# JuliaQuantumControl/GRAPE.jl

Measured on AMD Instinct MI355X. Metric: GRAPE gradient evals/sec (N=64, 1000 steps, 128 traj), higher is better.
Workload: dtype f64

## Files before the change

### grape.jl_amd/api.py

```python
from __future__ import annotations

import ctypes as C
import os
import subprocess
import sys

import numpy as np

_HERE = os.path.dirname(os.path.abspath(__file__))
_CSRC = os.path.join(_HERE, "csrc")
_LIBNAME = "libgrape_hip.so"

J_T_SM, J_T_SS, J_T_RE = 0, 1, 2
GRAD_GRADGEN, GRAD_TAYLOR = 0, 1
PROP_EXP, PROP_SERIES = 0, 1
ABI_VERSION = 7

STATUS = {0: "GRAPE_OK", -1: "GRAPE_ERR_INVALID", -2: "GRAPE_ERR_HIP", -3: "GRAPE_ERR_CHI_NORM",
          -4: "GRAPE_ERR_SINGULAR", -5: "GRAPE_ERR_TAYLOR", -6: "GRAPE_ERR_NO_CONTROLS", -7: "GRAPE_ERR_AGAIN",
          -8: "GRAPE_ERR_HOST"}

EXPORTS = ["grape_create", "grape_destroy", "grape_eval", "grape_forward", "grape_backward",
           "grape_forward_device", "grape_backward_device", "grape_check", "grape_get_propagator",
           "grape_get_tau_grads", "grape_get_storage", "grape_get_timings", "grape_reset_timings", "grape_get_work", "grape_get_cert_table",
# ... 384 lines not shown

    def hvp_forward(self, V, final_states=False):
        v, nv = self._hvp_dirs(V)
        dtau = np.empty((nv, self.K), dtype=np.complex128)
        dsums = np.empty(nv, dtype=np.complex128)
        dpsi = np.empty((nv, self.K, self.N), dtype=np.complex128) if final_states else None
        self._chk(self._lib.grape_hvp_forward(self._h, nv, v.ctypes.data, dtau.ctypes.data, dsums.ctypes.data,
                                              dpsi.ctypes.data if final_states else None))
        if v.ndim == 1:
            dtau, dsums, dpsi = dtau[0], dsums[0], (dpsi[0] if final_states else None)
        return (dtau, dsums, dpsi) if final_states else (dtau, dsums)

    def hvp_backward(self, f_total, df_total):
        one = np.ndim(df_total) == 0
        df = np.ascontiguousarray(df_total, dtype=np.complex128)
        if np.ndim(df_total) > 1 or df.size == 0:
            raise ValueError(f"df_total must be a complex scalar or [nv] with nv >= 1, got {np.shape(df_total)}")
        nv = df.size
        out = np.empty((nv, self.L * self.N_T))
        f = np.array([complex(f_total).real, complex(f_total).imag], dtype=np.float64)
        self._chk(self._lib.grape_hvp_backward(self._h, nv, f.ctypes.data, df.ctypes.data, out.ctypes.data))
        return out[0] if one else out

    def hvp_backward_chi(self, chi, dchi):
        chi = np.ascontiguousarray(chi, dtype=np.complex128)
        d = np.ascontiguousarray(dchi, dtype=np.complex128)
        if chi.shape != (self.K, self.N):
            raise ValueError(f"chi must be [K, N] = [{self.K}, {self.N}], got {chi.shape}")
        if d.ndim not in (2, 3) or d.shape[-2:] != (self.K, self.N) or d.size == 0:
            raise ValueError(f"dchi must be [K, N] = [{self.K}, {self.N}] or [nv, {self.K}, {self.N}] with nv >= 1, got {d.shape}")
        nv = 1 if d.ndim == 2 else d.shape[0]
        out = np.empty((nv, self.L * self.N_T))
        self._chk(self._lib.grape_hvp_backward_chi(self._h, nv, chi.ctypes.data, d.ctypes.data, out.ctypes.data))
        return out[0] if d.ndim == 2 else out

    def set_tlist(self, tlist):
        t = np.ascontiguousarray(tlist, dtype=np.float64)
        if t.shape != (self.N_T + 1,):
            raise ValueError(f"tlist must have N_T + 1 = {self.N_T + 1} points, got {t.shape}")
        self._chk(self._lib.grape_set_tlist(self._h, t.ctypes.data))
        self._tlist = t

    def forward_device(self, d_pulsevals_ptr, d_out_ptr, stream=0):
        self._chk(self._lib.grape_forward_device(self._h, d_pulsevals_ptr, d_out_ptr, stream))

    def backward_device(self, d_f_ptr, d_G_ptr, stream=0):
        self._chk(self._lib.grape_backward_device(self._h, d_f_ptr, d_G_ptr, stream))

    def set_fused_sweeps(self, on=True):
        return bool(self._lib.grape_set_fused_sweeps(self._h, int(bool(on))))

    def check(self, stream=0):
        self._chk(self._lib.grape_check(self._h, stream))

    def propagator(self, k, n):
        out = np.empty((self.N, self.N), dtype=np.complex128)
        self._chk(self._lib.grape_get_propagator(self._h, k, n, out.ctypes.data))
        return out.T.copy()

    def tau_grads(self):
        out = np.empty((self.K, self.L, self.N_T), dtype=np.complex128)
        self._chk(self._lib.grape_get_tau_grads(self._h, out.ctypes.data))
        return out

    def storage(self, which=0):
        out = np.empty((self.K, self.N_T + 1, self.N), dtype=np.complex128)
        self._chk(self._lib.grape_get_storage(self._h, which, out.ctypes.data))
        return out

    def timings(self):
        ms = np.full(8, -1.0)
        self._lib.grape_get_timings(self._h, ms.ctypes.data, 8)
        out = dict(zip(["expm", "forward", "backward", "deriv", "reduce", "total"], ms[:6].tolist()))
        if ms[6] >= 0.0:
            out["host_enqueue"] = float(ms[6])
        if ms[7] >= 0.0:
            out["gradient_allreduce_us"] = float(ms[7]) * 1e3
        return out

    def reset_timings(self):
        self._chk(self._lib.grape_reset_timings(self._h))

    def work(self):
        w = np.zeros(20)
        self._lib.grape_get_work(self._h, w.ctypes.data, 20)
        return dict(cells=w[0], squarings=w[1], flop_expm=w[2], flop_deriv=w[3], deriv_orders=w[4],
                    pivoted_cells=w[5], expm_cells=w[6], series_terms=w[7], series_steps=w[8],
                    t18_mfma_flop=w[9], t18_squarings=w[10], t18_cells=w[11], matrix_free_fallback=w[12], t16_cells=w[13],
                    asm_kernel=w[14], asm_deriv_kernel=w[15], asm_blocked_products=w[16],
                    walk_steps=w[17], scan_block=w[18], t16_certified=w[19])

    def cert_table(self):
        dims = np.zeros(3, np.int32)
        self._chk(self._lib.grape_get_cert_table(self._h, dims.ctypes.data, None, None))
        KC, n8, n6 = (int(x) for x in dims)
        coef, exps = np.zeros((KC, n8 + n6)), np.zeros(n8 + n6, np.int32)
        if n8 + n6:
            self._chk(self._lib.grape_get_cert_table(self._h, dims.ctypes.data, coef.ctypes.data, exps.ctypes.data))
        ex = np.stack([(exps >> (4 * l)) & 15 for l in range(self.L)], axis=1) if n8 + n6 else np.zeros((0, self.L), np.int32)
        return coef[:, :n8], coef[:, n8:], ex


def liouvillian(H, cops=()):
    H = np.asarray(H, dtype=np.complex128)
    d = H.shape[0]
    if H.shape != (d, d):
        raise ValueError(f"H must be [d, d], got {H.shape}")
    eye = np.eye(d)
    heff = H.copy()
    for A in cops:
        A = np.asarray(A, dtype=np.complex128)
        heff = heff - 0.5j * (A.conj().T @ A)
    out = np.kron(eye, heff) - np.kron(heff.conj(), eye)
    for A in cops:
        A = np.asarray(A, dtype=np.complex128)
        out = out + 1j * np.kron(A.conj(), A)
    return out


class GrapeHipOpen(GrapeHip):

    def __init__(self, H0, Hc, cops, tlist, rho0, target, weights=None, functional=J_T_SM, shape=None, K_total=None,
                 device=0, chi_min_norm=0.0, prop_tolerance=0.0):
        self._lib = load_library()
        H0 = np.asarray(H0)
        if H0.ndim != 3 or H0.shape[1] != H0.shape[2]:
            raise ValueError(f"H0 must be [K, d, d], got {H0.shape}")
        K, N = H0.shape[0], H0.shape[1]
        Hc = np.asarray(Hc)
        per_traj = Hc.ndim == 4
        if Hc.ndim not in (3, 4) or Hc.shape[-2:] != (N, N) or (per_traj and Hc.shape[0] != K):
            raise ValueError(f"Hc must be [L, d, d] or [K, L, d, d] with d = {N}, K = {K}, got {Hc.shape}")
        L = Hc.shape[1] if per_traj else Hc.shape[0]
        tlist = np.ascontiguousarray(tlist, dtype=np.float64)
        if tlist.ndim != 1 or len(tlist) < 2:
            raise ValueError("tlist must hold at least two time points")
        N_T = len(tlist) - 1
        if weights is not None and np.shape(weights) != (K,):
            raise ValueError(f"weights must be [K] = [{K}], got {np.shape(weights)}")
        cops = None if cops is None or np.size(cops) == 0 else np.asarray(cops)
        cops_per_traj = cops is not None and cops.ndim == 4
        if cops is not None and (cops.ndim not in (3, 4) or cops.shape[-2:] != (N, N) or (cops_per_traj and cops.shape[0] != K)):
            raise ValueError(f"cops must be [J, d, d] or [K, J, d, d] with d = {N}, K = {K}, got {cops.shape}")
        self.N, self.L, self.K, self.N_T = N, L, K, N_T
        self.J = 0 if cops is None else cops.shape[-3]
        self.K_total = K if K_total is None else int(K_total)
        self.functional = functional
        self.prop_method = PROP_EXP
        self.lambda_b = 0.0
        self._H0 = _c128(np.swapaxes(H0, -1, -2), (K, N, N))
        self._Hc = _c128(np.swapaxes(Hc, -1, -2))
        self._cops = None if cops is None else _c128(np.swapaxes(cops, -1, -2))
        self._psi0 = _c128(np.swapaxes(np.asarray(rho0), -1, -2), (K, N, N))
        self._target = None if target is None else _c128(np.swapaxes(np.asarray(target), -1, -2), (K, N, N))
        self._tlist = tlist
        self._weights = None if weights is None else np.ascontiguousarray(weights, dtype=np.float64)
        self._shape = None if shape is None else np.ascontiguousarray(shape, dtype=np.float64).reshape(L, N_T)
        p = _Problem()
        p.abi_version = ABI_VERSION
        p.N, p.L, p.K, p.K_total, p.N_T = N, L, K, self.K_total, N_T
        p.functional, p.gradient_method, p.hc_per_traj, p.device = functional, GRAD_GRADGEN, int(per_traj), device
        p.tlist = self._tlist.ctypes.data
        p.H0 = self._H0.ctypes.data
        p.Hc = self._Hc.ctypes.data
        p.shape = None if self._shape is None else self._shape.ctypes.data
        p.psi0 = self._psi0.ctypes.data
        p.target = None if self._target is None else self._target.ctypes.data
        p.weights = None if self._weights is None else self._weights.ctypes.data
        p.chi_min_norm = chi_min_norm
        p.prop_method, p.prop_tolerance = PROP_EXP, float(prop_tolerance)
        d = _Lindblad()
        d.J, d.cops_per_traj = self.J, int(cops_per_traj)
        d.cops = None if self._cops is None else self._cops.ctypes.data
# ... 114 lines not shown
```

### grape.jl_amd/csrc/grape_hip.hip

```cpp
#include "../../include/grape_hip.h"
#include "grape_kernels.hip.h"
#include "grape_t18_coeffs.h"
#include "grape_econ_coeffs.h"
#include "grape_large.hip.h"
#include "grape_series.hip.h"
#include "grape_cheby.hip.h"
#include "grape_timegrad.hip.h"
#include "grape_lindblad.hip.h"
#include "grape_lindblad_tg.hip.h"
#include "grape_hvp.hip.h"
#include "grape_hvp_split.hip.h"
#include "grape_lindblad_hvp.hip.h"
#include "grape_lindblad_batch.hip.h"
#include "grape_lindblad_rc.hip.h"
#include "grape_devmem.h"
#include "grape_cert.hip.h"

#include <rccl/rccl.h>
#include <dlfcn.h>
#include <mutex>

#include <algorithm>
#include <chrono>
#include <cmath>
// ... 15 lines not shown
        *err = std::string("host-side C++ exception caught at the C boundary: ") + what;
    } catch (...) {
    }
    return -8;
}
#define GRAPE_BARRIER(errptr)                                                                                   \
    catch (const std::bad_alloc &) { return barrier_fail((errptr), "std::bad_alloc (out of host memory)"); }    \
    catch (const std::exception &e) { return barrier_fail((errptr), e.what()); }                                \
    catch (...) { return barrier_fail((errptr), "unknown exception"); }

void test_throw_point(const char *where) {
    const char *hk = getenv("GRAPE_TEST_HOOKS");
    if (!(hk && atoi(hk) == 1)) return;
    const char *t = getenv("GRAPE_TEST_THROW"), *at = getenv("GRAPE_TEST_THROW_AT");
    if (!t || strcmp(at ? at : "early", where)) return;
    if (!strcmp(t, "bad_alloc")) throw std::bad_alloc();
    throw std::runtime_error(t);
}

constexpr int kRing = 64;
constexpr int kPhases = 6;
struct Phase { hipEvent_t e0, e1; bool used; };

}

struct OpenCtx;

struct grape_handle {
    grape_problem p{};
    int N = 0, NP = 0, NT = 0, L = 0, K = 0, K_total = 0, N_T = 0;
    int device = 0;
    hipStream_t stream = nullptr;
    double *d_H0f = nullptr, *d_Hcf = nullptr, *d_H0t = nullptr, *d_Hct = nullptr;
    double *d_H0p = nullptr, *d_Hcp = nullptr, *d_vecs = nullptr;
    double *d_H0q = nullptr, *d_Hcq = nullptr, *d_park2 = nullptr;
    double *d_H0q3 = nullptr, *d_Hcq3 = nullptr, *d_H0p3 = nullptr, *d_Hcp3 = nullptr;
    int deriv4_blocks = 0;
    double *d_park3 = nullptr;
    int deriv3_blocks = 0, deriv3_wpt = 0;
    bool deriv3_h0g = false;
    bool deriv3_general = false;
    int deriv2 = 0, deriv2_maxm = 0;
    bool deriv_stream = false;
    bool deriv_stream_never = false;
    int deriv_blocks = 0;
    bool large = false;
    int chunk = 0;
    double *d_lg[9] = {nullptr, nullptr, nullptr, nullptr, nullptr, nullptr, nullptr, nullptr, nullptr};
    double *d_dinv = nullptr;
    int *d_scell = nullptr;
    double *d_colpart = nullptr;
    bool lg_form2 = false;
    double *d_normpart = nullptr;
    double *d_dts = nullptr, *d_shape = nullptr, *d_weights = nullptr;
    double2 *d_psi0 = nullptr, *d_target = nullptr;
    double *d_eps = nullptr;
    double2 *d_U = nullptr, *d_fw = nullptr, *d_bw = nullptr, *d_tg = nullptr;
    double *d_ret = nullptr;
    double *d_out = nullptr;
    double *d_f = nullptr, *d_G = nullptr, *d_rho = nullptr;
    int *d_flags = nullptr;
    int *d_cellflag = nullptr;
    int KC = 0;
    bool herm = false;
    bool herm_ctrl = false;
    bool t18 = false;
    bool t18_small = true;
    bool t16 = true;
    double *d_gram = nullptr;
    int *d_celllist = nullptr;
    double *d_cert = nullptr;
    int *d_cert_exp = nullptr;
    int cert_n8 = 0, cert_n6 = 0;
    bool asm16 = false;
    bool asm16p = false;
    double *d_dte = nullptr;
    bool asm18gp = false;
    bool asm18g = false;
    int *d_wgtab = nullptr, *d_prog = nullptr, *d_splan = nullptr;
    double2 *d_xinit = nullptr;
    int asm_blocks = 0;
    int last_walk_fuse = 0;
    bool asm_sq = true;
    int asm_walk = 0;
    bool foreign_stream = false;
    bool credit_pending = false;
    std::vector<double> bal;
    std::vector<double> bal_stage_chi, bal_stage_xi;
    double *d_Sf = nullptr;
    bool expm_persist = true;
    int expm_lds_pad_kb = 0;
    bool test_hooks = false;
    bool lg_asm = true;
    bool deriv3_asm = true;
    bool taylor_check = true;
    bool no_target = false;
    std::vector<int> cls;
    int *d_cls = nullptr, *d_rep = nullptr;
    int coop_S = 0;
    int *d_xcc_sw = nullptr;
    int coop_rpw = 0, coop_nw = 0;
    double2 *d_Dt = nullptr, *d_xi = nullptr;
    double *d_wq = nullptr, *d_gb = nullptr;
    bool have_gb = false;
    const double2 *xi_user = nullptr;
    double lambda_user = 0.0;
    unsigned long long *d_stats = nullptr;
    double *h_pin = nullptr;
    DeviceBufs mem;
    size_t h_pin_doubles = 0;
    Phase ph[kRing][kPhases]{};
    long n_fwd = 0, n_bwd = 0;
    std::string err;
    bool have_forward = false, in_eval = false;
    double chi_min_norm = 1e-100, taylor_tol = 1e-16;
    int taylor_max_order = 100;
    bool fuse = false;
    bool fuse_on = true;
    bool want_bw = true;
    bool bw_done = false;
    bool bw_unit = false;
    bool z_valid = false;
    double *d_inv_tnorm = nullptr, *d_ones = nullptr;
    double2 *d_z = nullptr;
    bool scan16 = false;
    int scan_Bk = 0, scan_NB = 0;
    double2 *d_scanF = nullptr, *d_scan_fw = nullptr, *d_scan_bw = nullptr;
    int num_cus = 256;
    bool series = false;
    bool u_fallback = false;
    double *d_rb = nullptr;
    double series_tol = 1e-17, series_theta = 3.0;
    double *d_n1 = nullptr;
    double2 *d_gpark = nullptr;
    int *d_morder = nullptr;
    int maxp = 0;
    int *d_batchflag = nullptr;
    bool deriv_econ = false;
    const double *d_econ_pairs = nullptr;
    int *d_celldeg = nullptr;
    double sub_theta = 0.0;
    int sq_plan = 2;
    double2 *d_xch = nullptr;
    int *d_xcc = nullptr;
    int cheby_S = 0, cheby_round = 0, cheby_pair = 0;
    double2 *d_chi_in = nullptr;
    std::vector<grape_handle *> shards;
    std::vector<int> shard_lo;
    std::vector<int> shard_dev;
    bool use_rccl = false;
    void *comm_set = nullptr;
    std::vector<double *> d_red;
    bool rccl_fwd_checked = false, rccl_bwd_checked = false;
    hipEvent_t ar0 = nullptr, ar1 = nullptr;
    double allreduce_ms = 0.0;
    long allreduce_calls = 0;
    std::vector<double> h_multi;
    bool multi_threads = true;
    double host_enqueue_ms = 0.0;
    long host_enqueue_calls = 0;
    bool graph_ok = false, capturing = false;
    hipGraph_t graph = nullptr;
    hipGraphExec_t graph_exec = nullptr;
    bool graph_fuse_on = true;
    bool graph_bw_unit = false, graph_z_valid = false, graph_credit = false;
    long n_eval = 0;
// ... 40 lines not shown
#define HIPCHK(h, expr)                                                                         \
    do {                                                                                        \
        hipError_t _e = (expr);                                                                 \
        if (_e != hipSuccess) {                                                                 \
            (h)->err = std::string(#expr) + ": " + hipGetErrorString(_e);                       \
            return GRAPE_ERR_HIP;                                                               \
        }                                                                                       \
    } while (0)

template <typename Layout>
int group_reserve(grape_handle *h, GroupStore &g, int want, size_t per, double budget_cap, const char *call, const char *unit_word,
                  const char *env_name, int *units, Layout &&layout, bool *grown = nullptr) {
    hipError_t e = g.plan(want, per, budget_cap, units);
    if (e != hipSuccess) { h->err = std::string("hipMemGetInfo(&free_b, &total_b): ") + hipGetErrorString(e); return GRAPE_ERR_HIP; }
    const GroupStore::Grow r = g.grow(*units, h->stream, layout, &e);
    if (grown) *grown = r == GroupStore::Grow::grown;
    if (r == GroupStore::Grow::sync_failed) { h->err = std::string("hipStreamSynchronize(h->stream): ") + hipGetErrorString(e); return GRAPE_ERR_HIP; }
    if (r == GroupStore::Grow::alloc_failed) {
        h->err = GroupStore::oom_message(call, *units, unit_word, per, env_name);
        (void)hipGetLastError();
        return GRAPE_ERR_HIP;
    }
    return GRAPE_OK;
}

int copy_info(const double *info, int len, double *out, int n) {
    const int m = std::max(0, std::min(n, len));
    for (int i = 0; i < m; ++i) out[i] = info[i];
    return m;
}

struct LdsLimit {
    size_t set[64] = {0};
    hipError_t ensure(const void *fn, int dev, size_t bytes) {
        size_t &cur = set[((unsigned)dev) % 64u];
        if (bytes <= cur) return hipSuccess;
        hipError_t e = hipFuncSetAttribute(fn, hipFuncAttributeMaxDynamicSharedMemorySize, (int)bytes);
        if (e == hipSuccess) cur = bytes;
        return e;
    }
};

size_t expm_lds_bytes(int NT) {
    const int total = NT == 1 ? ExpmLds<1>::TOTAL : NT == 2 ? ExpmLds<2>::TOTAL : NT == 3 ? ExpmLds<3>::TOTAL : ExpmLds<4>::TOTAL;
    return sizeof(double) * (size_t)total;
}

template <int NT>
hipError_t launch_expm(const ExpmArgs &a, bool herm, hipStream_t s, int persistent_blocks = 0, int lds_pad_kb = 0) {
    static LdsLimit lim_fast, lim_piv, lim_herm, lim_pers, lim_persh;
    const size_t lds = expm_lds_bytes(NT) + (size_t)lds_pad_kb * 1024;
    int dev = 0;
    hipGetDevice(&dev);
    {
        hipError_t e = lim_fast.ensure((const void *)expm_pade_kernel<NT, false>, dev, lds);
        if (e == hipSuccess) e = lim_piv.ensure((const void *)expm_pade_kernel<NT, true>, dev, lds);
        if (e == hipSuccess && NT >= 3) e = lim_herm.ensure((const void *)expm_pade_kernel<NT, false, NT >= 3>, dev, lds);
        if (e != hipSuccess) return e;
    }
    hipError_t e = hipMemsetAsync(a.cellflag, 0, (size_t)a.K * a.N_T * sizeof(int), s);
    if (e != hipSuccess) return e;
    if (NT == 4 && persistent_blocks > 0) {
        hipError_t ep = lim_pers.ensure((const void *)expm_persistent_kernel<NT, false>, dev, lds);
        if (ep == hipSuccess) ep = lim_persh.ensure((const void *)expm_persistent_kernel<NT, NT == 4>, dev, lds);
        if (ep != hipSuccess) return ep;
        if (herm) hipLaunchKernelGGL((expm_persistent_kernel<NT, NT == 4>), dim3(persistent_blocks), dim3(NT * 64), lds, s, a);
        else hipLaunchKernelGGL((expm_persistent_kernel<NT, false>), dim3(persistent_blocks), dim3(NT * 64), lds, s, a);
    } else
    if (herm && NT >= 3)
        hipLaunchKernelGGL((expm_pade_kernel<NT, false, NT >= 3>), dim3(a.K * a.N_T), dim3(NT * 64), lds, s, a);
    else
        hipLaunchKernelGGL((expm_pade_kernel<NT, false>), dim3(a.K * a.N_T), dim3(NT * 64), lds, s, a);
    hipLaunchKernelGGL((expm_pade_kernel<NT, true>), dim3(std::min(a.K * a.N_T, 1024)), dim3(NT * 64), lds, s, a);
    return hipGetLastError();
}

extern "C" int grape_t18_launch(int NT, int herm, int t16, const void *args, size_t args_size, void *stream, int blocks);
extern "C" const double *grape_econ_pairs(void);
extern "C" int grape_t16p_asm_launch(const void *args, size_t args_size, int *verdict, void *stream, int blocks,
                                     const void *const *walk, int fuse, int K, const double *dte);
extern "C" int grape_t18g_asm_launch(const void *args, size_t args_size, int *verdict, void *stream, int blocks,
                                     const void *const *walk, int fuse, int K, const double *dte);
extern "C" int grape_t16_asm_launch(const void *args, size_t args_size, int *verdict, void *stream, int blocks,
                                    const void *const *walk, int fuse, int K);
extern "C" int grape_t18_batch_launch(int herm, const void *args, size_t args_size, const void *strides, size_t strides_size,
                                      int sets, void *stream, int blocks);
extern "C" void grape_t16_walks(int KC, int N_T, int nblk, int *tab);
extern "C" int grape_t16_credit_launch(const void *args, size_t args_size, void *stream);
static bool deriv3_fits(int NT, int L, bool h0_general = false) {
    const size_t tile = (size_t)2 * 16 * 17 * sizeof(double), mat = (size_t)(NT * (NT + 1) / 2) * tile;
    if (h0_general) return NT >= 3 && NT <= 4 && L >= 1 && L <= 2 && (size_t)NT * NT * tile + (size_t)L * mat <= 160 * 1024;
    return L >= 1 && L <= 8 && (size_t)(1 + L) * mat <= 160 * 1024;
}
extern "C" int grape_deriv3_launch(int NT, const void *d2args, size_t d2size, const double *H0f, const double *Hcf, int wpt,
                                   int skip_if_flagged, int h0_general, int use_asm, void *stream, int blocks);
extern "C" int grape_lg_asm_launch(const void *k, size_t size, unsigned blocks, void *stream);
extern "C" int grape_deriv4_launch(int NP, const void *d2args, size_t d2size, const double *H0q3, const double *Hcq3, const double *H0p3,
                                   const double *Hcp3, void *stream, int blocks);
#ifdef GRAPE_DIAG
extern "C" void grape_t18_set_stamps(unsigned long long *d_stamps, void *stream);
#endif

template <int CPL>
hipError_t launch_coop(const SweepArgs &a, bool backward, int S, int rpw, int nw, hipStream_t s) {
    hipError_t e;
    if (a.xcc) {
        e = hipMemsetAsync(a.xcc, 0xFF, (size_t)a.K * 32 * sizeof(int), s);
        if (e != hipSuccess) return e;
    }
    e = hipMemsetAsync((void *)a.store, 0xFF, (size_t)a.K * (a.N_T + 1) * 64 * CPL * sizeof(double2), s);
    if (e != hipSuccess) return e;
    const dim3 grid(8 * ((a.K + 7) / 8) * S), block(64 * nw);
#define COOP_CASE(NW_, RPW_)                                                                                          \
    if (nw == NW_ && rpw == RPW_) {                                                                                   \
        if (backward) hipLaunchKernelGGL((sweep_coop_kernel<CPL, RPW_, NW_, true>), grid, block, 0, s, a, S);         \
        else hipLaunchKernelGGL((sweep_coop_kernel<CPL, RPW_, NW_, false>), grid, block, 0, s, a, S);                 \
        return hipGetLastError();                                                                                     \
    }
    COOP_CASE(4, 1) COOP_CASE(8, 1) COOP_CASE(16, 1) COOP_CASE(16, 2) COOP_CASE(16, 4)
#undef COOP_CASE
    return hipErrorInvalidValue;
}

static bool g_sweep_wg32 = false;
template <int NP>
hipError_t launch_sweep(const SweepArgs &a, bool backward, hipStream_t s);
template <int NP>
hipError_t launch_sweep_pair(const SweepArgs &af, const SweepArgs &ab, hipStream_t s);

template <int NT>
hipError_t launch_scan_block(const ScanArgs &sa, hipStream_t s) {
    static LdsLimit lim;
    constexpr int NP = 16 * NT;
    const size_t lds = (size_t)2 * 2 * NP * (NP + 2) * sizeof(double);
    int dev = 0;
    hipGetDevice(&dev);
    hipError_t e = lim.ensure((const void *)scan_block_kernel<NT>, dev, lds);
    if (e != hipSuccess) return e;
    hipLaunchKernelGGL((scan_block_kernel<NT>), dim3((unsigned)(sa.KC * sa.NB)), dim3(64 * NT), lds, s, sa);
    return hipGetLastError();
}

hipError_t launch_scan(grape_handle *h, const SweepArgs *af, const SweepArgs *ab, bool blocks, hipStream_t s) {
    const int NB = h->scan_NB, Bk = h->scan_Bk, NP = h->NP;
    const SweepArgs &any = af ? *af : *ab;
    hipError_t e = hipSuccess;
    if (blocks) {
        if (NP == 16) {
            Scan16Args sa{};
            sa.U = any.U; sa.F = h->d_scanF; sa.KC = h->KC; sa.N_T = any.N_T; sa.Bk = Bk; sa.NB = NB;
            hipLaunchKernelGGL(scan16_block_kernel, dim3((unsigned)(h->KC * NB)), dim3(64), 0, s, sa);
            e = hipGetLastError();
        } else {
            ScanArgs sa{};
            sa.U = any.U; sa.F = h->d_scanF; sa.KC = h->KC; sa.N_T = any.N_T; sa.Bk = Bk; sa.NB = NB;
            e = NP == 32 ? launch_scan_block<2>(sa, s) : NP == 48 ? launch_scan_block<3>(sa, s) : launch_scan_block<4>(sa, s);
        }
        if (e != hipSuccess) return e;
    }
    SweepArgs cf{}, cb{};
    if (af) { cf = *af; cf.U = h->d_scanF; cf.N_T = NB; cf.store = h->d_scan_fw; cf.resume = nullptr; }
    if (ab) { cb = *ab; cb.U = h->d_scanF; cb.N_T = NB; cb.store = h->d_scan_bw; cb.resume = nullptr; }
    if (af && ab) e = NP == 16 ? launch_sweep_pair<16>(cf, cb, s) : NP == 32 ? launch_sweep_pair<32>(cf, cb, s)
                      : NP == 48 ? launch_sweep_pair<48>(cf, cb, s) : launch_sweep_pair<64>(cf, cb, s);
    else {
        const SweepArgs &c1 = af ? cf : cb;
        const bool bw = !af;
// ... 778 lines not shown
    return ra;
}

hipError_t launch_cheby(grape_handle *h, const SweepArgs *sf, const SweepArgs *sb, hipStream_t s) {
    const int NP = h->NP, S = h->cheby_S, K = h->K;
    const size_t lds = sizeof(double) * ((size_t)2 * 16 * (NP + 2) + 2 * (size_t)NP + CHEBY_MAXT + 2);
    static LdsLimit lim;
    {
        hipError_t e = lim.ensure((const void *)cheby_coop_kernel, h->device, lds);
        if (e != hipSuccess) return e;
    }
    hipLaunchKernelGGL(cheby_arm_kernel, dim3(256), dim3(256), 0, s, (unsigned long long *)h->d_xch, (size_t)2 * K * 4 * NP * 2);
    hipError_t e = hipGetLastError();
    if (e != hipSuccess) return e;
    e = hipMemsetAsync(h->d_xcc, 0xFF, (size_t)2 * K * 32 * sizeof(int), s);
    if (e != hipSuccess) return e;
    auto fill = [&](ChebyArgs &c, const SweepArgs &sa, bool backward) {
        c.s = sa;
        c.H0 = backward ? h->d_H0t : h->d_H0f;
        c.Hc = backward ? h->d_Hct : h->d_Hcf;
        c.eps = h->d_eps; c.shape = h->d_shape; c.dts = h->d_dts; c.rb = h->d_rb; c.stats = h->d_stats;
        c.xch = h->d_xch + (backward ? (size_t)K * 4 * NP : 0);
        c.xcc = h->d_xcc + (backward ? (size_t)K * 32 : 0);
        c.tol = h->series_tol;
        c.L = h->L; c.hc_per_traj = h->p.hc_per_traj; c.NP = NP; c.herm = h->herm ? 1 : 0;
    };
    for (int k0 = 0; k0 < K; k0 += h->cheby_round) {
        const int kn = std::min(h->cheby_round, K - k0);
        ChebyArgs cf{}, cb{};
        if (sf) { fill(cf, *sf, false); cf.k0 = k0; cf.kn = kn; }
        if (sb) { fill(cb, *sb, true); cb.k0 = k0; cb.kn = kn; }
        const int nb = 8 * ((kn + 7) / 8) * S;
        if (sf && sb) hipLaunchKernelGGL(cheby_coop_kernel, dim3(2 * nb), dim3(256), lds, s, cf, cb, S, nb);
        else if (sf) { cb = cf; cb.kn = 0; hipLaunchKernelGGL(cheby_coop_kernel, dim3(nb), dim3(256), lds, s, cf, cb, S, nb); }
        else { cf = cb; hipLaunchKernelGGL(cheby_coop_kernel, dim3(nb), dim3(256), lds, s, cf, cb, S, 0); }
        e = hipGetLastError();
        if (e != hipSuccess) return e;
    }
    return hipSuccess;
}

int status_from_flags(grape_handle *h, int flags) {
    if (flags & 32) {
        h->err = "the squaring plan of the blocked exponential was too short for this evaluation; the plan has been "
                 "adapted: repeat the call (the host-pointer entry points do so themselves)";
        return GRAPE_ERR_AGAIN;
    }
    if (flags & 1) { h->err = "Pade denominator numerically singular in at least one cell"; return GRAPE_ERR_SINGULAR; }
    if (flags & 64) { h->err = "exponential: a generator H_kn dt is not finite (NaN or overflow)"; return GRAPE_ERR_SINGULAR; }
    if (flags & 2) {
        h->err = "The chi state of at least one trajectory has norm < chi_min_norm (optimize.jl:1021-1025)";
        return GRAPE_ERR_CHI_NORM;
    }
    if (flags & 8) { h->err = "cooperative sweep: a sibling workgroup did not arrive (spin limit reached)"; return GRAPE_ERR_HIP; }
    if (flags & 16) {
        h->err = "matrix-free propagator: the series of exp(-i H dt) did not converge within the order limit";
        return GRAPE_ERR_TAYLOR;
    }
    if (flags & 4) {
        const bool cut_at_the_limit = h->NP < 48 || h->taylor_max_order <= 64;
        const bool one_term = h->p.gradient_method == GRAPE_GRAD_TAYLOR && h->taylor_max_order <= 1;
        if ((h->taylor_check || !cut_at_the_limit) && !one_term) {
            h->err = h->taylor_check ? "taylor_grad_step! did not converge within max_order iterations (optimize.jl:644-648)"
                                     : "taylor_grad_check_convergence = false with taylor_max_order > 64: a series of this evaluation was "
                                       "still unconverged at the 64 terms the series kernels of N > 32 hold";
            return GRAPE_ERR_TAYLOR;
        }
    }
    return GRAPE_OK;
}

int multi_create(grape_handle **out, const grape_problem *p);
struct HandleGuard {
    grape_handle *h;
    explicit HandleGuard(grape_handle *h_) : h(h_) {}
    HandleGuard(const HandleGuard &) = delete;
    HandleGuard &operator=(const HandleGuard &) = delete;
    ~HandleGuard() { if (h) { grape_destroy(h); (void)hipGetLastError(); } }
    grape_handle *release() { grape_handle *r = h; h = nullptr; return r; }
};
thread_local const std::vector<double> *tl_forced_bal = nullptr;
int multi_fail(grape_handle *h, grape_handle *c, int rc);
int backward_device_impl(grape_handle *h, const double *d_f, double *d_G, hipStream_t s, const double2 *d_chi);
double open_lambda_b(const grape_handle *h);

double functional_from_sums(const grape_handle *h, const double *sums) {
    const double Kt = (double)h->K_total;
    double J;
    if (h->p.functional == GRAPE_J_T_SM) J = 1.0 - (sums[0] * sums[0] + sums[1] * sums[1]) / (Kt * Kt);
    else if (h->p.functional == GRAPE_J_T_SS) J = 1.0 - sums[2] / Kt;
    else J = 1.0 - sums[3] / Kt;
    if (h->open) { if (open_lambda_b(h) != 0.0) J += open_lambda_b(h) * sums[4]; }
    else if (h->p.Dpen && h->p.lambda_b != 0.0) J += h->p.lambda_b * sums[4];
    return J;
}


}

struct OpenCtx {
    int J = 0, cops_per_traj = 0, Kj = 1, Kc = 1;
    double *d_H0 = nullptr, *d_Hc = nullptr, *d_Dc = nullptr, *d_A = nullptr, *d_AdA = nullptr, *d_rho0 = nullptr, *d_target = nullptr,
           *d_chi = nullptr, *d_weights = nullptr, *d_eps = nullptr, *d_shape = nullptr, *d_dts = nullptr, *d_rb = nullptr,
           *d_store = nullptr, *d_ws = nullptr, *d_out = nullptr, *d_f = nullptr, *d_rho = nullptr, *d_G = nullptr;
    double2 *d_tg = nullptr;
    int *d_flags = nullptr;
    unsigned long long *d_stats = nullptr;
    DeviceBufs mem;
    hipEvent_t ev[2] = {nullptr, nullptr};
    double ms_fwd = 0.0, ms_bwd = 0.0;
    long n_fwd = 0, n_bwd = 0;
    std::vector<double> out;
    std::vector<double> stage;
    bool have_bwd = false;
    enum { TG_NONE, TG_NO_GRADIENT, TG_FORWARD_ONLY, TG_READY, TG_FAILED, TG_NEW_GRID, TG_BATCH, TG_NEW_COST, TG_RUNNING_COST };
    int tg_state = TG_NONE;
    bool tg_chi_user = false;
    size_t ws_mats = 0;
    double2 *d_tq = nullptr;
    double *d_dJdt = nullptr;
    enum { HV_NONE, HV_READY, HV_FAILED, HV_NEW_GRID, HV_BATCH, HV_NEW_COST };
    int hv_state = HV_NONE;
    struct HvpStore {
        GroupStore store;
        double *d_hvV = nullptr, *d_hvws = nullptr, *d_hvds = nullptr, *d_hvout = nullptr;
        double2 *d_hvdtau = nullptr, *d_hvdcoef = nullptr, *d_hvtg = nullptr;
        unsigned long long *d_hvstats = nullptr;
        double info[7] = {0., 0., 0., 0., 0., 0., 0.};
    } hv;
    struct BatchStore {
        GroupStore store;
        double *d_obeps = nullptr, *d_obstore = nullptr, *d_obws = nullptr, *d_obout = nullptr, *d_obrho = nullptr, *d_obG = nullptr;
        double2 *d_obtg = nullptr;
        int *d_obflags = nullptr;
        unsigned long long *d_obstats = nullptr;
        double info[7] = {0., 0., 0., 0., 0., 0., 0.};
    } ob;
    bool rc_set = false;
    int rc_per_traj = 0;
    double rc_lambda = 0.0;
    double *d_Xi = nullptr, *d_wq = nullptr, *d_gb = nullptr, *d_xi_user = nullptr;
    std::vector<double> tlist;
};

namespace {

template <typename T>
hipError_t open_alloc(OpenCtx *o, T **p, size_t n) { return o->mem.alloc(p, std::max<size_t>(n, 1)); }

double open_lambda_b(const grape_handle *h) { return h->open->rc_set ? h->open->rc_lambda : 0.0; }

void open_destroy(grape_handle *h) {
    OpenCtx *o = h->open;
    hipSetDevice(h->device);
    if (h->stream) hipStreamSynchronize(h->stream);
    o->hv.store.release(); o->ob.store.release(); o->mem.release();
    for (hipEvent_t e : o->ev)
        if (e) hipEventDestroy(e);
    if (h->stream) hipStreamDestroy(h->stream);
    delete o;
    delete h;
}

void open_to_planar(const double *src, int N, int NP, double *dst) {
    std::fill(dst, dst + 2 * (size_t)NP * NP, 0.0);
    for (int j = 0; j < N; ++j)
// ... 1132 lines not shown
        std::vector<double> rb((size_t)K + (size_t)Kc * L);
        const bool rigorous = h->herm && h->series && h->large;
        auto bound_of = [&](const double *m) { return rigorous ? herm_norm2_bound(m, N) : norm2_estimate(m, N); };
        const int nops = K + Kc * L;
        auto op_ptr = [&](int q) { return q < K ? p->H0 + 2 * (size_t)q * nn : p->Hc + 2 * (size_t)(q - K) * nn; };
        if (rigorous && nops > 1) {
            parallel_for(nops, [&](int q) { rb[q] = bound_of(op_ptr(q)); });
        } else {
            for (int q = 0; q < nops; ++q) rb[q] = bound_of(op_ptr(q));
        }
        CCHK(h->mem.alloc(&h->d_rb, rb.size()));
        CCHK(hipMemcpy(h->d_rb, rb.data(), rb.size() * 8, hipMemcpyHostToDevice));
        const char *envd = getenv("GRAPE_DERIV_THETA");
        h->sub_theta = p->gradient_method == GRAPE_GRAD_GRADGEN ? (envd ? atof(envd) : 4.0) : 0.0;
        CCHK(h->mem.alloc(&h->d_batchflag, (size_t)2 * K * ((N_T + 15) / 16)));
        CCHK(hipMemset(h->d_batchflag, 0, (size_t)2 * K * ((N_T + 15) / 16) * sizeof(int)));
    }
    if (h->series) {
        const char *env = getenv("GRAPE_SERIES_THETA");
        if (env && atof(env) > 0) h->series_theta = atof(env);
        const char *envp = getenv("GRAPE_SERIES_PARK");
        const size_t bytes = (size_t)K * N_T * 32 * NP * 16;
        size_t free_p = 0, total_p = 0;
        if (const char *envb = getenv("GRAPE_U_BUDGET_GB")) free_p = (size_t)(atof(envb) * 1073741824.0);
        else if (hipMemGetInfo(&free_p, &total_p) != hipSuccess) free_p = (size_t)-1;
        if (NP >= 48 && !h->large && h->deriv2 && h->series_tol <= h->taylor_tol && bytes <= ((size_t)24 << 30) &&
            (double)bytes <= 0.5 * (double)free_p && !(envp && atoi(envp) == 0)) {
            h->maxp = 32;
            CCHK(h->mem.alloc(&h->d_gpark, (size_t)K * N_T * h->maxp * NP));
            CCHK(h->mem.alloc(&h->d_morder, (size_t)K * N_T));
            CCHK(hipMemset(h->d_morder, 0xFF, (size_t)K * N_T * sizeof(int)));
        }
    }
    CCHK(h->mem.alloc(&h->d_fw, (size_t)K * (N_T + 1) * NP));
    CCHK(h->mem.alloc(&h->d_bw, (size_t)K * (N_T + 1) * NP));
    {
        const char *envs = getenv("GRAPE_SCAN16");
        if (const char *envs2 = getenv("GRAPE_SCAN")) envs = envs2;
        { const char *env1w = getenv("GRAPE_SWEEP1W"); g_sweep_wg32 = env1w && atoi(env1w) == 0; }
        const bool forced = envs && atoi(envs) != 0;
        const int kmax = NP == 16 ? 96 : NP == 32 ? 64 : NP == 48 ? 48 : 24;
        if (NP <= 64 && !h->series && !h->large && !(envs && atoi(envs) == 0) && N_T >= 8 && (forced || (h->KC <= kmax && N_T >= 64))) {
            const double t2 = NP == 16 ? 0.22 : NP == 32 ? 1.1 : 1.8, t1 = NP == 16 ? 0.45 : NP == 32 ? 3.3 : NP == 48 ? 7.3 : 13.5;
            const double slots = NP == 16 ? 16.0 * h->num_cus : (double)h->num_cus;
            int best = 4;
            double best_t = 1e300;
            for (int Bk = 4; Bk <= 64 && Bk < std::max(N_T, 5); Bk += (Bk < 16 ? 2 : 4)) {
                const int NBq = (N_T + Bk - 1) / Bk;
                const double t = std::ceil((double)h->KC * NBq / slots) * Bk * t1 + (NBq + Bk) * t2;
                if (t < best_t) { best_t = t; best = Bk; }
            }
            if (const char *envb = getenv("GRAPE_SCAN16_BK")) best = std::max(2, atoi(envb));
            h->scan_Bk = std::min(best, N_T);
            h->scan_NB = (N_T + h->scan_Bk - 1) / h->scan_Bk;
            CCHK(h->mem.alloc(&h->d_scanF, (size_t)h->KC * h->scan_NB * NP * NP));
            CCHK(h->mem.alloc(&h->d_scan_fw, (size_t)K * (h->scan_NB + 1) * NP));
            CCHK(h->mem.alloc(&h->d_scan_bw, (size_t)K * (h->scan_NB + 1) * NP));
            h->scan16 = true;
        }
    }
    CCHK(h->mem.alloc(&h->d_tg, (size_t)K * L * N_T));
    CCHK(h->mem.alloc(&h->d_ret, (size_t)2 * K + 8 + (size_t)L * N_T + 4 + (size_t)GRAPE_STAT_SHARDS * GRAPE_STAT_SLOTS));
    h->d_out = h->d_ret;
    h->d_G = h->d_ret + (size_t)2 * K + 8;
    h->d_flags = (int *)(h->d_G + (size_t)L * N_T);
    h->d_stats = (unsigned long long *)(h->d_G + (size_t)L * N_T + 4);
    CCHK(h->mem.alloc(&h->d_f, 2)); CCHK(h->mem.alloc(&h->d_rho, (size_t)K));
    CCHK(h->mem.alloc(&h->d_cellflag, (size_t)K * N_T));
    bool sf_per_cell_ok = false;
    const char *envp16 = getenv("GRAPE_EXPM_ASM16P");
    const bool p_direct = p->hc_per_traj && (h->herm ? L <= 4 : L <= 2) && !(envp16 && atoi(envp16) == 0);
    if (p->hc_per_traj && !p_direct && h->t18 && !h->large && !h->series && h->NT == 4) {
        size_t free_b = 0, total_b = 0;
        CCHK(hipMemGetInfo(&free_b, &total_b));
        const char *envs = getenv("GRAPE_SF_PER_CELL");
        sf_per_cell_ok = !(envs && atoi(envs) == 0) && 2.0 * (double)h->KC * N_T * NP * NP * 16.0 + 8e9 < (double)free_b;
    }
    const bool sf_shape_ok = !p->hc_per_traj || p_direct || sf_per_cell_ok;
    h->asm16 = h->asm16 && h->t16 && h->t18 && h->herm && !h->large && !h->series && h->NT == 4 && sf_shape_ok && (long)K * N_T < (1L << 28);
    h->asm18g = h->asm18g && h->t18 && !h->herm && !h->large && !h->series && h->NT == 4 && sf_shape_ok && (long)K * N_T < (1L << 28);
    h->asm16p = h->asm16 && p_direct;
    h->asm18gp = h->asm18g && p_direct;
    {
        const char *enve = getenv("GRAPE_DERIV_ECON");
        const bool lg_ok = h->large && h->t18 && h->herm && !h->series;
        const bool t16c_ok = h->t16 && h->t18 && h->herm && !h->large && !h->series && (h->NT >= 3 || (h->NT == 2 && h->t18_small));
        h->deriv_econ = (h->asm16 || lg_ok || t16c_ok) && p->gradient_method == GRAPE_GRAD_GRADGEN && h->taylor_tol >= 1e-16 && h->d_batchflag &&
                        !(enve && atoi(enve) == 0);
        if (h->deriv_econ) h->d_econ_pairs = grape_econ_pairs();
        if (h->deriv_econ && !h->d_econ_pairs) h->deriv_econ = false;
        if (h->deriv_econ && lg_ok) {
            CCHK(h->mem.alloc(&h->d_celldeg, (size_t)h->KC * N_T));
            CCHK(hipMemset(h->d_celldeg, 0, (size_t)h->KC * N_T * sizeof(int)));
        }
    }
    if (h->asm16p || h->asm18gp) CCHK(h->mem.alloc(&h->d_dte, (size_t)(L <= 2 ? 4 : 8) * N_T));
    if (h->t18 && !h->large && !h->series && ((L > 2 && !p->hc_per_traj) || (h->asm16 && !h->asm16p) || (h->asm18g && !h->asm18gp)) && (h->NT >= 3 || h->t18_small))
        CCHK(h->mem.alloc(&h->d_Sf, (size_t)(p->hc_per_traj ? (size_t)h->KC * N_T : (size_t)N_T) * 2 * NP * NP));
    if (h->asm16 || h->asm18g) {
        const long ncell = (long)h->KC * N_T;
        h->asm_blocks = (int)std::max<long>(1, std::min<long>(h->num_cus, ncell));
        std::vector<int> tab((size_t)4 * h->asm_blocks);
        grape_t16_walks(h->KC, N_T, h->asm_blocks, tab.data());
        CCHK(h->mem.alloc(&h->d_wgtab, tab.size()));
        CCHK(h->mem.alloc(&h->d_splan, (size_t)ncell));
        CCHK(hipMemset(h->d_splan, 0, (size_t)ncell * sizeof(int)));
        CCHK(hipMemcpy(h->d_wgtab, tab.data(), tab.size() * sizeof(int), hipMemcpyHostToDevice));
        const char *envw = getenv("GRAPE_EXPM_WALK"), *envq = getenv("GRAPE_EXPM_SQ");
        h->asm_sq = !(envq && atoi(envq) == 0);
        h->asm_walk = h->KC == K ? (envw ? atoi(envw) & 3 : 3) : 0;
        if (h->scan16) h->asm_walk = 0;
        if (h->asm_walk) {
            std::vector<double> xi((size_t)2 * K * 64 * 2, 0.0);
            for (int k = 0; k < K; ++k) {
                double n2 = 0.0;
                for (int i = 0; i < 2 * N; ++i) n2 += p->target[(size_t)k * 2 * N + i] * p->target[(size_t)k * 2 * N + i];
                const double itn = n2 > 0.0 ? 1.0 / std::sqrt(n2) : 0.0;
                for (int i = 0; i < N; ++i) {
                    xi[2 * ((size_t)k * 64 + i)] = p->psi0[2 * ((size_t)k * N + i)];
                    xi[2 * ((size_t)k * 64 + i) + 1] = p->psi0[2 * ((size_t)k * N + i) + 1];
                    xi[2 * ((size_t)(K + k) * 64 + i)] = p->target[2 * ((size_t)k * N + i)] * itn;
                    xi[2 * ((size_t)(K + k) * 64 + i) + 1] = -p->target[2 * ((size_t)k * N + i) + 1] * itn;
                }
            }
            CCHK(h->mem.alloc(&h->d_xinit, (size_t)2 * K * 64));
            CCHK(hipMemcpy(h->d_xinit, xi.data(), xi.size() * 8, hipMemcpyHostToDevice));
            CCHK(h->mem.alloc(&h->d_prog, (size_t)2 * K));
            CCHK(hipMemset(h->d_prog, 0, (size_t)2 * K * sizeof(int)));
        }
    }
    if (h->t16 && h->t18 && h->herm && !h->large && !h->series && (h->NT >= 3 || (h->NT == 2 && h->t18_small))) {
        CCHK(h->mem.alloc(&h->d_celllist, (size_t)K * N_T));
        const int M = L + 1, KCn = h->KC;
        const int GS = M * M + M;
        std::vector<double> gram((size_t)KCn * GS);
        std::vector<int> repk(KCn, -1);
        auto shape_factor = [&](const double *op, double fro2) {
            if (!(fro2 > 0.0)) return 1.0;
            std::vector<double> a2((size_t)2 * N * N), a4((size_t)2 * N * N);
            auto square = [&](const double *a, std::vector<double> &c) {
                std::fill(c.begin(), c.end(), 0.0);
                for (int j = 0; j < N; ++j)
                    for (int k = 0; k < N; ++k) {
                        const double br = a[2 * ((size_t)j * N + k)], bi = a[2 * ((size_t)j * N + k) + 1];
                        const double *ak = a + 2 * (size_t)k * N;
                        double *cj = &c[2 * (size_t)j * N];
                        for (int i = 0; i < N; ++i) {
                            cj[2 * i] += ak[2 * i] * br - ak[2 * i + 1] * bi;
                            cj[2 * i + 1] += ak[2 * i] * bi + ak[2 * i + 1] * br;
                        }
                    }
            };
            square(op, a2);
            square(a2.data(), a4);
            double m8 = 0.0;
            for (double x : a4) m8 += x * x;
            const double s8 = std::pow(m8, 0.125), semi = std::pow(3.5, 0.125) * 2.0 * std::sqrt(fro2 / (double)N);
            const double kap = s8 / semi;
            return std::isfinite(kap) && kap > 0.0 ? kap : 1.0;
        };
        std::vector<double> kap_shared((size_t)L, -1.0);
        for (int k = K - 1; k >= 0; --k) repk[h->cls.empty() ? k : h->cls[k]] = k;
        const size_t nn2 = (size_t)2 * N * N;
        for (int kc = 0; kc < KCn; ++kc) {
            const int k = repk[kc] < 0 ? kc : repk[kc];
            auto op = [&](int a) { return a == 0 ? p->H0 + (size_t)k * nn2 : p->Hc + ((size_t)(p->hc_per_traj ? k : 0) * L + (a - 1)) * nn2; };
// ... 70 lines not shown
        int S = 1;
        while (S * 2 * groups <= per_xcd && h->NP / (S * 2) >= 4) S *= 2;
        const int R = h->NP / S;
        const char *env = getenv("GRAPE_SWEEP_COOP");
        if (S >= 2 && R <= 64 && !(env && atoi(env) == 0)) {
            h->coop_S = S;
            h->coop_nw = R >= 16 ? 16 : R;
            h->coop_rpw = R / h->coop_nw;
            CCHK(h->mem.alloc(&h->d_xcc_sw, (size_t)2 * K * 32));
        }
    }
    CCHK(hipMemset(h->d_flags, 0, 8 * sizeof(int)));
    CCHK(hipMemset(h->d_stats, 0, (size_t)GRAPE_STAT_SHARDS * GRAPE_STAT_SLOTS * sizeof(unsigned long long)));
    CCHK(hipMemset(h->d_fw, 0, (size_t)K * (N_T + 1) * NP * 16));
    CCHK(hipMemset(h->d_bw, 0, (size_t)K * (N_T + 1) * NP * 16));
    CCHK(hipMemset(h->d_tg, 0, (size_t)K * L * N_T * 16));
    h->h_pin_doubles = (size_t)2 * L * N_T + 2 * K + 16;
    if (p->Dpen && p->lambda_b != 0.0) {
        h->have_gb = true;
        const int Kd = p->dpen_per_traj ? K : 1;
        std::vector<double> dt_((size_t)Kd * pp * 2, 0.0);
        for (int kd = 0; kd < Kd; ++kd)
            for (int j = 0; j < N; ++j)
                for (int i = 0; i < N; ++i) {
                    dt_[2 * ((size_t)kd * pp + (size_t)j * NP + i)] = p->Dpen[2 * ((size_t)kd * nn + (size_t)j * N + i)];
                    dt_[2 * ((size_t)kd * pp + (size_t)j * NP + i) + 1] = p->Dpen[2 * ((size_t)kd * nn + (size_t)j * N + i) + 1];
                }
        CCHK(h->mem.alloc(&h->d_Dt, (size_t)Kd * pp));
        CCHK(hipMemcpy(h->d_Dt, dt_.data(), dt_.size() * 8, hipMemcpyHostToDevice));
        std::vector<double> wq(N_T + 1);
        for (int m = 0; m <= N_T; ++m)
            wq[m] = m == 0 ? (p->tlist[1] - p->tlist[0]) / 2.0
                           : (m < N_T ? 0.5 * (p->tlist[m + 1] - p->tlist[m - 1]) : (p->tlist[N_T] - p->tlist[N_T - 1]) / 2.0);
        CCHK(h->mem.alloc(&h->d_wq, (size_t)N_T + 1));
        CCHK(hipMemcpy(h->d_wq, wq.data(), wq.size() * 8, hipMemcpyHostToDevice));
        CCHK(h->mem.alloc(&h->d_xi, (size_t)K * (N_T + 1) * NP));
        CCHK(h->mem.alloc(&h->d_gb, (size_t)K * (N_T + 1)));
    }
    {
        h->batch_ok = !h->large && !h->series && NP == 16 && h->t18 && h->t18_small && p->gradient_method == GRAPE_GRAD_GRADGEN &&
                      !h->have_gb && h->fuse && !h->no_target && h->K == h->K_total && !h->test_hooks && L <= 8;
        if (const char *envb = getenv("GRAPE_BATCH")) h->batch_env = atoi(envb) != 0 ? 1 : 0;
        if (const char *envs = getenv("GRAPE_BATCH_SETS")) h->batch.store.env = std::max(0, atoi(envs));
        if (const char *envh = getenv("GRAPE_HVP_DIRS")) h->hvp.store.env = std::max(0, atoi(envh));
    }
    CCHK(h->mem.alloc_pinned(&h->h_pin, h->h_pin_doubles));
    CCHK(hipDeviceSynchronize());
#undef CCHK
    test_throw_point("late");
    *out = guard.release();
    return GRAPE_OK;
}
GRAPE_BARRIER(&g_create_error)

int grape_forward_device(grape_handle *h, const double *d_pulsevals, double *d_out, void *stream_) try {
    if (h && h->open) return open_refuse(h, "grape_forward_device");
    if (!h || !d_pulsevals || !d_out) return GRAPE_ERR_INVALID;
    if (!h->shards.empty()) { h->err = "device-pointer entry points need a single-device handle (ndev <= 1)"; return GRAPE_ERR_INVALID; }
    hipStream_t s = (hipStream_t)stream_;
    h->foreign_stream = s != h->stream;
    HIPCHK(h, hipSetDevice(h->device));
    (void)hipGetLastError();
    HIPCHK(h, hipMemsetAsync(h->d_flags, 0, 8 * sizeof(int) + (size_t)GRAPE_STAT_SHARDS * GRAPE_STAT_SLOTS * sizeof(unsigned long long), s));
    if (d_pulsevals != h->d_eps)
        HIPCHK(h, hipMemcpyAsync(h->d_eps, d_pulsevals, (size_t)h->L * h->N_T * 8, hipMemcpyDeviceToDevice, s));
    ExpmArgs ea{};
    ea.H0f = h->d_H0f; ea.Hcf = h->d_Hcf; ea.eps = h->d_eps; ea.shape = h->d_shape; ea.dts = h->d_dts;
    ea.U = h->d_U; ea.flags = h->d_flags; ea.stats = h->d_stats; ea.cellflag = h->d_cellflag;
    ea.K = h->KC; ea.rep = h->d_rep; ea.L = h->L; ea.N_T = h->N_T; ea.hc_per_traj = h->p.hc_per_traj;
    ea.n1 = h->d_n1; ea.n1_k = h->K;
#ifdef GRAPE_DIAG
    ea.ablate = getenv("GRAPE_DIAG_ABLATE") ? atoi(getenv("GRAPE_DIAG_ABLATE")) : 0;
    static unsigned long long *d_stamps = nullptr;
    if (getenv("GRAPE_DIAG_STAMPS")) {
        if (!d_stamps) hipMalloc((void **)&d_stamps, (size_t)h->K * h->N_T * 32 * 8);
        hipMemsetAsync(d_stamps, 0, (size_t)h->K * h->N_T * 32 * 8, s);
    }
    ea.stamps = d_stamps;
    hipMemcpyToSymbolAsync(HIP_SYMBOL(g_diag_slot_base), &d_stamps, sizeof(d_stamps), 0, hipMemcpyHostToDevice, s);
    grape_t18_set_stamps(d_stamps, (void *)s);
#endif
    hipError_t e = hipSuccess;
    int walk_fuse = 0;
    if (!h->series) {
        phase_begin(h, 0, s);
        if (h->large) {
            e = h->t18 ? expm_large_t18(h, s) : expm_large(h, s);
        } else {
            const long ncell = (long)ea.K * ea.N_T;
            const int per_cu = h->NT == 1 ? 10 : h->NT == 2 ? 4 : 1;
            const int t18_blocks = 8 * (int)std::max<long>(1, std::min<long>((long)(h->num_cus / 8) * per_cu, (ncell + 7) / 8));
            if (h->t18 && (h->NT >= 3 || h->t18_small)) {
                if (h->d_Sf) {
                    CtrlSumArgs ca{};
                    ca.Hcf = h->d_Hcf; ca.eps = h->d_eps; ca.shape = h->d_shape; ca.Sf = h->d_Sf;
                    ca.L = h->L; ca.N_T = h->N_T; ca.pp2 = 2 * h->NP * h->NP;
                    ca.per_traj = h->p.hc_per_traj ? 1 : 0; ca.rep = h->d_rep;
                    hipLaunchKernelGGL(ctrl_sum_kernel, dim3((unsigned)((ca.per_traj ? h->KC : 1) * h->N_T), std::max(1, ca.pp2 / 2 / 2048)), dim3(256), 0, s, ca);
                    HIPCHK(h, hipGetLastError());
                    ea.Sf = h->d_Sf;
                }
                const bool t16 = h->d_celllist != nullptr;
                ea.cell_list = h->d_celllist; ea.listed = 0;
                if (t16) {
                    T16PlanArgs pa{};
                    pa.gram = h->d_gram; pa.eps = h->d_eps; pa.shape = h->d_shape; pa.dts = h->d_dts; pa.flags = h->d_flags;
                    pa.KC = h->KC; pa.L = h->L; pa.N_T = h->N_T; pa.N = h->N;
                    pa.splan = (h->asm16 && (h->asm_sq || h->d_cert)) ? h->d_splan : nullptr;
                    pa.sq_on = h->asm_sq ? 1 : 0;
                    pa.cert = h->d_cert; pa.cert_exp = h->d_cert_exp; pa.n8 = h->cert_n8; pa.n6 = h->cert_n6;
                    pa.verdict = h->d_cellflag;
                    hipLaunchKernelGGL(t16_plan_kernel, dim3((unsigned)((ncell + 255) / 256)), dim3(256), 0, s, pa);
                    HIPCHK(h, hipGetLastError());
                }
                const int blocks16 = (t16 && h->NT == 3) ? 8 * (int)std::max<long>(1, std::min<long>((long)(h->num_cus / 8) * 2, (ncell + 7) / 8)) : t18_blocks;
                h->credit_pending = false;
                if (h->asm18g) {
                    walk_fuse = h->asm_walk & (1 | ((h->fuse && h->fuse_on && h->want_bw) ? 2 : 0));
                    if (walk_fuse) HIPCHK(h, hipMemsetAsync(h->d_prog, 0, (size_t)2 * h->K * sizeof(int), s));
                    const void *walk[6] = {h->d_wgtab, h->d_xinit, h->d_fw, h->d_bw, h->d_prog, h->d_splan};
                    if (h->asm18gp) {
                        hipLaunchKernelGGL(dte_kernel, dim3((unsigned)((h->N_T + 255) / 256)), dim3(256), 0, s, (const double *)h->d_eps,
                                           (const double *)h->d_shape, (const double *)h->d_dts, h->L, h->N_T, 2, h->d_dte);
                        HIPCHK(h, hipGetLastError());
                    }
                    e = (hipError_t)grape_t18g_asm_launch(&ea, sizeof(ea), h->d_cellflag, (void *)s, h->asm_blocks, walk, walk_fuse, h->K,
                                                          h->asm18gp ? h->d_dte : nullptr);
                    h->credit_pending = !h->asm18gp;
                }
                else if (t16 && h->asm16p) {
                    walk_fuse = h->asm_walk & (1 | ((h->fuse && h->fuse_on && h->want_bw) ? 2 : 0));
                    if (walk_fuse) HIPCHK(h, hipMemsetAsync(h->d_prog, 0, (size_t)2 * h->K * sizeof(int), s));
                    hipLaunchKernelGGL(dte_kernel, dim3((unsigned)((h->N_T + 255) / 256)), dim3(256), 0, s, (const double *)h->d_eps,
                                       (const double *)h->d_shape, (const double *)h->d_dts, h->L, h->N_T, h->L <= 2 ? 2 : 4, h->d_dte);
                    HIPCHK(h, hipGetLastError());
                    const void *walk[6] = {h->d_wgtab, h->d_xinit, h->d_fw, h->d_bw, h->d_prog, h->d_splan};
                    e = (hipError_t)grape_t16p_asm_launch(&ea, sizeof(ea), h->d_cellflag, (void *)s, h->asm_blocks, walk, walk_fuse, h->K, h->d_dte);
                }
                else if (t16 && h->asm16) {
                    walk_fuse = h->asm_walk & (1 | ((h->fuse && h->fuse_on && h->want_bw) ? 2 : 0));
                    if (walk_fuse) HIPCHK(h, hipMemsetAsync(h->d_prog, 0, (size_t)2 * h->K * sizeof(int), s));
                    const void *walk[6] = {h->d_wgtab, h->d_xinit, h->d_fw, h->d_bw, h->d_prog, h->d_splan};
                    e = (hipError_t)grape_t16_asm_launch(&ea, sizeof(ea), h->d_cellflag, (void *)s, h->asm_blocks, walk, walk_fuse, h->K);
                    h->credit_pending = true;
                }
                else
                    e = (hipError_t)grape_t18_launch(h->NT, h->herm ? 1 : 0, t16 ? 1 : 0, &ea, sizeof(ea), (void *)s, blocks16);
                if (t16 && e == hipSuccess) {
                    ea.listed = 1;
                    e = (hipError_t)grape_t18_launch(h->NT, 1, 0, &ea, sizeof(ea), (void *)s, t18_blocks);
                }
            } else
            switch (h->NT) {
                case 1: e = launch_expm<1>(ea, h->herm, s, 0, h->expm_lds_pad_kb); break;
                case 2: e = launch_expm<2>(ea, h->herm, s, 0, h->expm_lds_pad_kb); break;
                case 3: e = launch_expm<3>(ea, h->herm, s, 0, h->expm_lds_pad_kb); break;
                default: {
                    const int nb = 8 * (h->num_cus / 8);
                    const bool persist = h->expm_persist && nb >= 8 && (long)ea.K * ea.N_T >= 4L * nb;
                    e = launch_expm<4>(ea, h->herm, s, persist ? nb : 0, h->expm_lds_pad_kb);
                    break;
                }
            }
        }
        HIPCHK(h, e);
        if (h->deriv_econ) {
            DerivEconArgs ec{};
            ec.verdict = h->d_cellflag; ec.splan = h->d_splan; ec.cls = h->d_cls; ec.flags = h->d_flags;
            ec.cell_deg = h->large ? h->d_celldeg : nullptr;
            ec.deg0 = ECON_DEG[0]; ec.deg1 = ECON_DEG[ECON_NSETS - 1];
            static_assert(ECON_NSETS == 4, "segments 1.36 (verdict), 1.6, 2.0 (blocked path), 2.72 (one planned squaring)");
            ec.K = h->K; ec.KC = h->KC; ec.N_T = h->N_T; ec.batches_per_k = (h->N_T + 15) / 16;
            ec.nbatch_total = h->K * ec.batches_per_k; ec.batch_econ = h->d_batchflag + ec.nbatch_total;
            hipLaunchKernelGGL(deriv_econ_kernel, dim3((unsigned)((ec.nbatch_total + 255) / 256)), dim3(256), 0, s, ec);
            HIPCHK(h, hipGetLastError());
        }
        phase_end(h, 0, s);
    }
#ifdef GRAPE_DIAG
    if (ea.stamps) {
        hipStreamSynchronize(s);
        const size_t nb = (size_t)h->KC * h->N_T;
        std::vector<unsigned long long> st(nb * 32);
        hipMemcpy(st.data(), ea.stamps, nb * 32 * 8, hipMemcpyDeviceToHost);
        auto avg = [&](int i1, int i0) {
            double sum = 0;
            size_t cnt = 0;
            for (size_t b = 0; b < nb; ++b)
                if (st[b * 32 + i1] && st[b * 32 + i0]) { sum += (double)(st[b * 32 + i1] - st[b * 32 + i0]); ++cnt; }
            return cnt ? sum / cnt : 0.0;
        };
        if (h->t18 && h->NT >= 3) {
            const char *tn[] = {"form A (+norm)", "A2 = A A + half exchange", "A3 = A A2", "store A3, norm A2, barrier", "A6 = A3 A3",
                                "A6 exchanges + norms", "scaling, B1 -> X, barrier", "A9 = B1 B5", "+B4, B3+A9 -> X, B2", "p = B2 + (B3+A9) A9",
                                "squarings", "store U", "end barrier"};
            for (int j = 0; j < 13; ++j) fprintf(stderr, "  stamp %-28s %9.0f cycles\n", tn[j], avg(j + 1, j));
            fprintf(stderr, "  stamp %-28s %9.0f cycles\n", "TOTAL per cell", avg(13, 0));
        } else {
        const char *pn[] = {"form A", "norm", "A2", "A4,A6 (+store A2)", "store A6 + combos", "dual", "U=A*T"};
        for (int j = 0; j < 7; ++j) fprintf(stderr, "  stamp %-24s %9.0f cycles\n", pn[j], avg(11 + j, j ? 10 + j : 0));
        fprintf(stderr, "  stamp %-24s %9.0f cycles\n", "P,Q + first inversion", avg(5, 17));
        fprintf(stderr, "  stamp   barrier %6.0f, P/Q stores %6.0f, barrier %6.0f, strip loads + barrier + I_0 %6.0f\n", avg(26, 17), avg(27, 26), avg(28, 27), avg(5, 28));
        fprintf(stderr, "  stamp   strip loads + barrier %6.0f, then wave 0 (I_0) %6.0f, wave 1 (tiles + prefetch) %6.0f, wave 2 (prefetch) %6.0f\n", avg(22, 28), avg(29, 22), avg(30, 22), avg(31, 22));
        for (int j = 0; j < 4; ++j) fprintf(stderr, "  stamp solve step %d             %9.0f cycles\n", j, avg(6 + j, 5 + j));
        for (int j = 0; j < 1; ++j)
            fprintf(stderr, "  stamp   step %d, waves done after %6.0f %6.0f %6.0f %6.0f cycles\n", j, avg(18 + 4 * j, 5 + j),
                    avg(19 + 4 * j, 5 + j), avg(20 + 4 * j, 5 + j), avg(21 + 4 * j, 5 + j));
        fprintf(stderr, "  stamp %-24s %9.0f cycles\n", "squarings + store U", avg(4, 3));
        fprintf(stderr, "  stamp %-24s %9.0f cycles\n", "TOTAL per cell", avg(4, 0));
        }
    }
#endif
    h->last_walk_fuse = walk_fuse;
    h->tg_state = h->want_bw ? 2 : 1;
    h->hvs.came(grape_handle::HvpSplit::EVAL);
    SweepArgs sa{};
    sa.U = h->d_U; sa.cls = h->d_cls; sa.psi0 = h->d_psi0; sa.target = h->d_target; sa.weights = h->d_weights;
    sa.store = h->d_fw; sa.tau = (double2 *)d_out; sa.f = nullptr; sa.rho = h->d_rho; sa.flags = h->d_flags;
    sa.chi_min_norm = h->chi_min_norm;
    sa.K = h->K; sa.K_total = h->K_total; sa.N = h->N; sa.N_T = h->N_T; sa.functional = h->p.functional;
    sa.xcc = h->d_xcc_sw;
    if (walk_fuse & 1) sa.resume = h->d_prog;
    if (h->test_hooks) {
        const char *envd = getenv("GRAPE_TEST_DROP_SIBLING");
        sa.drop_sibling = envd ? atoi(envd) : 0;
    }
    phase_begin(h, 1, s);
    const bool pair = h->fuse && h->fuse_on && h->want_bw;
    h->bw_done = h->bw_unit = pair;
    h->z_valid = false;
    if (pair) {
        SweepArgs sb = sa;
        sb.store = h->d_bw; sb.tau = (double2 *)h->d_out; sb.f = nullptr; sb.unit_chi = 1; sb.inv_tnorm = h->d_inv_tnorm;
        sb.resume = (walk_fuse & 2) ? h->d_prog + h->K : nullptr;
        if (h->series && h->large) {
            e = launch_cheby(h, &sa, &sb, s);
        } else if (h->series) {
            const SeriesArgs rf = series_args(h, sa, false), rb = series_args(h, sb, true);
            const bool sc = 2 * h->K > h->num_cus;
            e = h->NP == 16 ? launch_series_pair<16>(rf, rb, sc, s) : h->NP == 32 ? launch_series_pair<32>(rf, rb, sc, s)
                                                                                 : launch_series_pair<64>(rf, rb, sc, s);
        } else if (h->scan16) {
            e = launch_scan(h, &sa, &sb, true, s);
        } else {
            e = h->NP == 16 ? launch_sweep_pair<16>(sa, sb, s) : h->NP == 32 ? launch_sweep_pair<32>(sa, sb, s)
                : h->NP == 48 ? launch_sweep_pair<48>(sa, sb, s) : launch_sweep_pair<64>(sa, sb, s);
        }
    } else if (h->series && h->large) {
        e = launch_cheby(h, &sa, nullptr, s);
    } else if (h->series) {
        const SeriesArgs ra = series_args(h, sa, false);
        e = h->NP == 16 ? launch_series<16>(ra, false, s) : h->NP == 32 ? launch_series<32>(ra, false, s)
                                                                       : launch_series<64>(ra, false, s);
    } else if (h->scan16) {
        e = launch_scan(h, &sa, nullptr, true, s);
    } else
    switch (h->NP) {
        case 16: e = launch_sweep<16>(sa, false, s); break;
        case 32: e = launch_sweep<32>(sa, false, s); break;
        case 48: e = launch_sweep<48>(sa, false, s); break;
        case 64: e = launch_sweep<64>(sa, false, s); break;
        default:
            if (h->coop_S)
                e = h->NP == 128 ? launch_coop<2>(sa, false, h->coop_S, h->coop_rpw, h->coop_nw, s)
                                 : launch_coop<4>(sa, false, h->coop_S, h->coop_rpw, h->coop_nw, s);
            else {
                hipLaunchKernelGGL((sweep_lg_kernel<false>), dim3(sa.K), dim3(1024), 0, s, sa, h->NP);
                e = hipGetLastError();
            }
    }
    HIPCHK(h, e);
    hipLaunchKernelGGL(tau_reduce_kernel, dim3(1), dim3(64), 0, s, (const double2 *)d_out, h->d_weights, h->K,
                       d_out + 2 * (size_t)h->K);
    HIPCHK(h, hipGetLastError());
    if (h->no_target) HIPCHK(h, hipMemsetAsync(d_out, 0xFF, ((size_t)2 * h->K + 4) * 8, s));
    if (h->have_gb) {
        GbArgs ga{};
        ga.Dt = h->d_Dt; ga.fw = h->d_fw; ga.xi = h->d_xi; ga.gb = h->d_gb;
        ga.NP = h->NP; ga.N_T = h->N_T; ga.d_per_traj = h->p.dpen_per_traj;
        hipLaunchKernelGGL(gb_kernel, dim3(h->K * (h->N_T + 1)), dim3(256), 0, s, ga);
        hipLaunchKernelGGL(jb_reduce_kernel, dim3(1), dim3(256), 0, s, (const double *)h->d_gb, (const double *)h->d_wq,
                           h->K, h->N_T, d_out + 2 * (size_t)h->K + 4);
        HIPCHK(h, hipGetLastError());
    }
    phase_end(h, 1, s);
    if (d_out != h->d_out)
        HIPCHK(h, hipMemcpyAsync(h->d_out, d_out, ((size_t)2 * h->K + 8) * 8, hipMemcpyDeviceToDevice, s));
    h->have_forward = true;
    if (!h->in_eval) h->n_fwd++;
    return GRAPE_OK;
}
GRAPE_BARRIER(h ? &h->err : &g_create_error)

int grape_backward_device(grape_handle *h, const double *d_f, double *d_G, void *stream_) try {
    if (h && h->open) return open_refuse(h, "grape_backward_device");
    if (!h || !d_f || !d_G) return GRAPE_ERR_INVALID;
    if (h->no_target) { h->err = "this handle has no target states (grape_problem.target == NULL): the built-in chi does not exist, use grape_backward_chi"; return GRAPE_ERR_INVALID; }
    if (!h->shards.empty()) { h->err = "device-pointer entry points need a single-device handle (ndev <= 1)"; return GRAPE_ERR_INVALID; }
    return backward_device_impl(h, d_f, d_G, (hipStream_t)stream_, nullptr);
}
GRAPE_BARRIER(h ? &h->err : &g_create_error)

}

namespace {
int backward_device_impl(grape_handle *h, const double *d_f, double *d_G, hipStream_t s, const double2 *d_chi) {
    if (!h->have_forward) { h->err = "grape_backward called before grape_forward"; return GRAPE_ERR_INVALID; }
    HIPCHK(h, hipSetDevice(h->device));
    (void)hipGetLastError();
    hipError_t e;
    SweepArgs sa{};
    sa.U = h->d_U; sa.cls = h->d_cls; sa.psi0 = h->d_psi0; sa.target = h->d_target; sa.weights = h->d_weights;
    sa.store = h->d_bw; sa.tau = (double2 *)h->d_out; sa.f = d_f; sa.rho = h->d_rho; sa.flags = h->d_flags;
    sa.xi = h->xi_user ? h->xi_user : (h->have_gb ? h->d_xi : nullptr); sa.wq = h->d_wq;
    sa.lambda_b = h->xi_user ? h->lambda_user : h->p.lambda_b;
    sa.chi_min_norm = h->chi_min_norm;
    sa.K = h->K; sa.K_total = h->K_total; sa.N = h->N; sa.N_T = h->N_T; sa.functional = h->p.functional;
    sa.xcc = h->d_xcc_sw ? h->d_xcc_sw + (size_t)h->K * 32 : nullptr;
    sa.chi_in = d_chi;
    phase_begin(h, 2, s);
    const bool unit = h->bw_done && !d_chi && !h->xi_user;
    h->bw_done = false;
    if (d_chi || h->xi_user) h->bw_unit = false;
    if (unit) {
        ChiCoeffArgs ca{};
        ca.s = sa; ca.s.inv_tnorm = h->d_inv_tnorm; ca.rho = h->d_rho; ca.z = h->d_z;
        hipLaunchKernelGGL(chi_coeff_kernel, dim3((h->K + 63) / 64), dim3(64), 0, s, ca);
        e = hipGetLastError();
        h->z_valid = true;
    } else if (h->series && h->large) {
        e = launch_cheby(h, nullptr, &sa, s);
    } else if (h->series) {
        const SeriesArgs ra = series_args(h, sa, true);
        e = h->NP == 16 ? launch_series<16>(ra, true, s) : h->NP == 32 ? launch_series<32>(ra, true, s)
                                                                      : launch_series<64>(ra, true, s);
    } else if (h->scan16 && !sa.xi) {
        e = launch_scan(h, nullptr, &sa, false, s);
    } else
    switch (h->NP) {
        case 16: e = launch_sweep<16>(sa, true, s); break;
        case 32: e = launch_sweep<32>(sa, true, s); break;
        case 48: e = launch_sweep<48>(sa, true, s); break;
        case 64: e = launch_sweep<64>(sa, true, s); break;
        default:
            if (h->coop_S)
                e = h->NP == 128 ? launch_coop<2>(sa, true, h->coop_S, h->coop_rpw, h->coop_nw, s)
                                 : launch_coop<4>(sa, true, h->coop_S, h->coop_rpw, h->coop_nw, s);
            else {
                hipLaunchKernelGGL((sweep_lg_kernel<true>), dim3(sa.K), dim3(1024), 0, s, sa, h->NP);
                e = hipGetLastError();
            }
    }
    HIPCHK(h, e);
    phase_end(h, 2, s);
    DerivArgs da{};
    da.H0t = h->d_H0t; da.Hct = h->d_Hct; da.eps = h->d_eps; da.shape = h->d_shape; da.dts = h->d_dts;
    da.fw = h->d_fw; da.bw = h->d_bw; da.rho = unit ? h->d_ones : h->d_rho; da.tg = h->d_tg; da.flags = h->d_flags; da.stats = h->d_stats;
    da.K = h->K; da.L = h->L; da.N_T = h->N_T; da.hc_per_traj = h->p.hc_per_traj;
    da.max_order = h->taylor_max_order; da.tol = h->taylor_tol;
    da.rb = h->d_rb; da.rb_k = h->K; da.sub_theta = h->sub_theta;
    int cpb = 16;
    while (cpb > 1 && (long)h->K * ((h->N_T + cpb - 1) / cpb) < 2048) cpb >>= 1;
    da.cells_per_block = cpb;
    const int nblocks = h->K * ((h->N_T + cpb - 1) / cpb);
    phase_begin(h, 3, s);
    if (h->NP >= 48 && h->sub_theta > 0.0) {
        HIPCHK(h, hipMemsetAsync(h->d_flags + 3, 0, sizeof(int), s));
        DerivFlagArgs fa{};
        fa.rb = h->d_rb; fa.eps = h->d_eps; fa.shape = h->d_shape; fa.dts = h->d_dts;
        fa.rb_k = h->K; fa.K = h->K; fa.L = h->L; fa.N_T = h->N_T; fa.hc_per_traj = h->p.hc_per_traj;
        fa.batches_per_k = (h->N_T + 15) / 16; fa.nbatch_total = h->K * fa.batches_per_k;
        fa.sub_theta = h->sub_theta; fa.batch_flag = h->d_batchflag; fa.flags = h->d_flags;
        hipLaunchKernelGGL(deriv_flag_kernel, dim3((fa.nbatch_total + 255) / 256), dim3(256), 0, s, fa);
        HIPCHK(h, hipGetLastError());
    }
    if (h->NP >= 48 && h->deriv2) {
        Deriv2Args d2{};
        d2.H0p = h->d_H0p; d2.Hcp = h->d_Hcp; d2.H0q = h->d_H0q; d2.Hcq = h->d_Hcq;
        d2.eps = h->d_eps; d2.shape = h->d_shape; d2.dts = h->d_dts;
        d2.fw = h->d_fw; d2.bw = h->d_bw; d2.rho = unit ? h->d_ones : h->d_rho; d2.tg = h->d_tg; d2.park = h->d_park2;
        d2.flags = h->d_flags; d2.stats = h->d_stats;
        d2.K = h->K; d2.L = h->L; d2.N_T = h->N_T; d2.hc_per_traj = h->p.hc_per_traj;
        d2.max_order = h->taylor_max_order; d2.maxm = h->deriv2_maxm; d2.tol = h->taylor_tol;
        d2.batches_per_k = (h->N_T + 15) / 16;
        d2.nbatch_total = h->K * d2.batches_per_k;
        if (h->series) { d2.gpark = h->d_gpark; d2.morder = h->d_morder; d2.maxp = h->maxp; }
        if (h->sub_theta > 0.0) d2.batch_flag = h->d_batchflag;
#ifdef GRAPE_DIAG
        d2.ablate = getenv("GRAPE_DIAG_ABLATE_D2") ? atoi(getenv("GRAPE_DIAG_ABLATE_D2")) : 0;
#endif
        if (h->d_park3 && !d2.gpark) {
            d2.park = h->d_park3;
            if (h->deriv_econ && !h->deriv3_general && !h->deriv3_h0g) {
                d2.batch_flag = h->d_batchflag;
                d2.batch_econ = 1; d2.econ_pairs = h->d_econ_pairs;
            }
            e = (hipError_t)grape_deriv3_launch(h->NT, &d2, sizeof(d2), h->d_H0f, h->d_Hcf, h->deriv3_wpt, 0, h->deriv3_general ? 2 : (h->deriv3_h0g ? 1 : 0), h->deriv3_asm ? 1 : 0, (void *)s, h->deriv3_blocks);
        } else if (h->deriv4_blocks && !d2.gpark) {
            if (h->deriv_econ && h->d_celldeg) {
                d2.batch_flag = h->d_batchflag;
                d2.batch_econ = 1; d2.econ_pairs = h->d_econ_pairs;
            }
            e = (hipError_t)grape_deriv4_launch(h->NP, &d2, sizeof(d2), h->d_H0q3, h->d_Hcq3, h->d_H0p3, h->d_Hcp3, (void *)s, h->deriv4_blocks);
        } else {
            if (h->deriv_econ && !d2.gpark && !h->large && h->herm) {
                d2.batch_flag = h->d_batchflag;
                d2.batch_econ = 1; d2.econ_pairs = h->d_econ_pairs;
            }
            e = launch_deriv2(h->NP, d2, h->deriv_blocks, s, h->deriv_stream, h->deriv_stream_never);
        }
    } else if (h->NP >= 48) {
        DerivMfmaArgs dm{};
        dm.H0p = h->d_H0p; dm.Hcp = h->d_Hcp; dm.eps = h->d_eps; dm.shape = h->d_shape; dm.dts = h->d_dts;
        dm.fw = h->d_fw; dm.bw = h->d_bw; dm.rho = unit ? h->d_ones : h->d_rho; dm.tg = h->d_tg; dm.vecs = h->d_vecs;
        dm.flags = h->d_flags; dm.stats = h->d_stats;
        dm.K = h->K; dm.L = h->L; dm.N_T = h->N_T; dm.hc_per_traj = h->p.hc_per_traj;
        dm.max_order = h->taylor_max_order; dm.tol = h->taylor_tol;
        dm.batches_per_k = (h->N_T + 15) / 16;
        dm.nbatch_total = h->K * dm.batches_per_k;
        if (h->sub_theta > 0.0) dm.batch_flag = h->d_batchflag;
        e = launch_deriv_mfma(h->NP, dm, h->deriv_blocks, s);
    } else {
        bool deep = false;
        if (h->d_park3) {
            Deriv2Args d2{};
            d2.eps = h->d_eps; d2.shape = h->d_shape; d2.dts = h->d_dts;
            d2.fw = h->d_fw; d2.bw = h->d_bw; d2.rho = unit ? h->d_ones : h->d_rho; d2.tg = h->d_tg; d2.park = h->d_park3;
            d2.flags = h->d_flags; d2.stats = h->d_stats;
            d2.K = h->K; d2.L = h->L; d2.N_T = h->N_T; d2.hc_per_traj = h->p.hc_per_traj;
            d2.max_order = h->taylor_max_order; d2.maxm = h->deriv2_maxm; d2.tol = h->taylor_tol;
            d2.batches_per_k = (h->N_T + 15) / 16;
            d2.nbatch_total = h->K * d2.batches_per_k;
            const bool sub = h->sub_theta > 0.0;
            d2.deep_redo = (!sub && h->taylor_max_order > h->deriv2_maxm) ? 1 : 0;
            if (h->deriv_econ && h->herm && h->NT == 2) {
                d2.batch_flag = h->d_batchflag;
                d2.batch_econ = 1; d2.econ_pairs = h->d_econ_pairs;
            }
            if (sub) {
                HIPCHK(h, hipMemsetAsync(h->d_flags + 3, 0, sizeof(int), s));
                DerivFlagArgs fa{};
                fa.rb = h->d_rb; fa.eps = h->d_eps; fa.shape = h->d_shape; fa.dts = h->d_dts;
                fa.rb_k = h->K; fa.K = h->K; fa.L = h->L; fa.N_T = h->N_T; fa.hc_per_traj = h->p.hc_per_traj;
                fa.batches_per_k = d2.batches_per_k; fa.nbatch_total = d2.nbatch_total;
                fa.sub_theta = h->sub_theta; fa.batch_flag = h->d_batchflag; fa.flags = h->d_flags;
                hipLaunchKernelGGL(deriv_flag_kernel, dim3((fa.nbatch_total + 255) / 256), dim3(256), 0, s, fa);
                HIPCHK(h, hipGetLastError());
            }
            HIPCHK(h, (hipError_t)grape_deriv3_launch(h->NT, &d2, sizeof(d2), h->d_H0f, h->d_Hcf, h->deriv3_wpt, sub ? 1 : 0, 0, h->deriv3_asm ? 1 : 0, (void *)s,
                                                      h->deriv3_blocks));
            da.only_if = sub ? h->d_flags + 3 : nullptr;
            if (d2.deep_redo) { deep = true; da.only_if = h->d_flags + 7; }
        }
        if (!h->d_park3 || h->sub_theta > 0.0 || deep) {
            switch (h->NP) {
                case 16: e = launch_deriv<16>(da, nblocks, s); break;
                default: e = launch_deriv<32>(da, nblocks, s); break;
            }
        }
    }
    HIPCHK(h, e);
    if (h->NP >= 48 && h->sub_theta > 0.0) {
        DerivSubArgs ds{};
        DerivMfmaArgs &dm = ds.m;
        dm.H0p = h->d_H0p; dm.Hcp = h->d_Hcp; dm.eps = h->d_eps; dm.shape = h->d_shape; dm.dts = h->d_dts;
        dm.fw = h->d_fw; dm.bw = h->d_bw; dm.rho = unit ? h->d_ones : h->d_rho; dm.tg = h->d_tg; dm.vecs = h->d_vecs;
        dm.flags = h->d_flags; dm.stats = h->d_stats;
        dm.K = h->K; dm.L = h->L; dm.N_T = h->N_T; dm.hc_per_traj = h->p.hc_per_traj;
        dm.max_order = h->taylor_max_order; dm.tol = h->taylor_tol;
        dm.batches_per_k = (h->N_T + 15) / 16;
        dm.nbatch_total = h->K * dm.batches_per_k;
        ds.rb = h->d_rb; ds.rb_k = h->K; ds.sub_theta = h->sub_theta; ds.batch_flag = h->d_batchflag;
        HIPCHK(h, launch_deriv_sub(h->NP, ds, h->deriv_blocks, s));
    }
    phase_end(h, 3, s);
    phase_begin(h, 4, s);
    const int LN = h->L * h->N_T;
    hipLaunchKernelGGL(grad_reduce_kernel, dim3((LN + 15) / 16), dim3(256), 0, s, h->d_tg, h->K, LN, d_G,
                       unit ? (const double2 *)h->d_z : (const double2 *)nullptr);
    HIPCHK(h, hipGetLastError());
    phase_end(h, 4, s);
    if (!h->capturing) h->n_bwd++;
    h->tg_state = 3; h->tg_unit = unit; h->tg_xi_user = h->xi_user != nullptr;
    return GRAPE_OK;
}
}

namespace {
int *pinned_flags(grape_handle *h) {
    return (int *)(h->h_pin + (size_t)2 * h->L * h->N_T + 2 * (size_t)h->K + 8);
}
int digest_flags(grape_handle *h, const int *flags) {
    if (h->large && !h->series) h->sq_plan = std::max(2, flags[1] + 1);
    return status_from_flags(h, flags[0]);
}

}

extern "C" {

int grape_set_fused_sweeps(grape_handle *h, int on) try {
    if (!h) return GRAPE_ERR_INVALID;
    if (h->open) return 0;
    if (!h->shards.empty()) {
        int r = 1;
        for (grape_handle *c : h->shards) r &= grape_set_fused_sweeps(c, on);
        return r;
    }
    h->fuse_on = on != 0;
    return (h->fuse && h->fuse_on) ? 1 : 0;
}
GRAPE_BARRIER(h ? &h->err : &g_create_error)

int grape_check(grape_handle *h, void *stream_) try {
    if (!h) return GRAPE_ERR_INVALID;
    if (h->open) {
        HIPCHK(h, hipSetDevice(h->device));
        HIPCHK(h, hipStreamSynchronize(h->stream));
        return GRAPE_OK;
    }
    if (!h->shards.empty()) {
        for (grape_handle *c : h->shards) {
            const int rc = grape_check(c, c->stream);
            if (rc) { h->err = c->err; return rc; }
        }
        return GRAPE_OK;
    }
    int *flags = pinned_flags(h);
    HIPCHK(h, hipSetDevice(h->device));
    HIPCHK(h, hipMemcpyAsync(flags, h->d_flags, 8 * sizeof(int), hipMemcpyDeviceToHost, (hipStream_t)stream_));
    HIPCHK(h, hipStreamSynchronize((hipStream_t)stream_));
    return digest_flags(h, flags);
}
GRAPE_BARRIER(h ? &h->err : &g_create_error)

}

namespace {

int forward_enqueue(grape_handle *h, const double *pulsevals, bool copy_out = true) {
    HIPCHK(h, hipSetDevice(h->device));
    const size_t nl = (size_t)h->L * h->N_T;
    memcpy(h->h_pin, pulsevals, nl * 8);
    HIPCHK(h, hipMemcpyAsync(h->d_eps, h->h_pin, nl * 8, hipMemcpyHostToDevice, h->stream));
    const int rc = grape_forward_device(h, h->d_eps, h->d_out, h->stream);
    if (rc) return rc;
    if (copy_out)
        HIPCHK(h, hipMemcpyAsync(h->h_pin + nl, h->d_out, ((size_t)2 * h->K + 8) * 8, hipMemcpyDeviceToHost, h->stream));
    return GRAPE_OK;
}
int forward_finish(grape_handle *h, double *tau) {
    const int rc = grape_check(h, h->stream);
    if (rc) return rc;
    if (tau) memcpy(tau, h->h_pin + (size_t)h->L * h->N_T, (size_t)2 * h->K * 8);
    return GRAPE_OK;
}
const double *forward_sums(const grape_handle *h) { return h->h_pin + (size_t)h->L * h->N_T + 2 * (size_t)h->K; }

int backward_enqueue(grape_handle *h, const double f_total[2], const double *chi, const double *xi = nullptr,
                     double lambda_b = 0.0, bool copy_out = true) {
    HIPCHK(h, hipSetDevice(h->device));
    if (!h->bal.empty()) {
// ... 542 lines not shown
        return GRAPE_ERR_INVALID;
    }
    HIPCHK(h, hipSetDevice(h->device));
    HIPCHK(h, hipDeviceSynchronize());
    const size_t pp = (size_t)h->NP * h->NP;
    std::vector<double> tmp(2 * pp);
    HIPCHK(h, hipMemcpy(tmp.data(), h->d_U + ((size_t)h->cls[k] * h->N_T + n) * pp, pp * 16, hipMemcpyDeviceToHost));
    for (int j = 0; j < h->N; ++j)
        for (int i = 0; i < h->N; ++i) {
            const double f = h->bal.empty() ? 1.0 : h->bal[i] / h->bal[j];
            out[2 * ((size_t)j * h->N + i)] = f * tmp[2 * ((size_t)i * h->NP + j)];
            out[2 * ((size_t)j * h->N + i) + 1] = f * tmp[2 * ((size_t)i * h->NP + j) + 1];
        }
    return GRAPE_OK;
}
GRAPE_BARRIER(h ? &h->err : &g_create_error)

int grape_get_timings(grape_handle *h, double *ms, int n) try {
    if (!h || !ms) return GRAPE_ERR_INVALID;
    if (h->open) {
        const OpenCtx *o = h->open;
        const double f = o->n_fwd ? o->ms_fwd / o->n_fwd : -1.0, b = o->n_bwd ? o->ms_bwd / o->n_bwd : -1.0;
        const double v[kPhases] = {0.0, f, b, 0.0, 0.0, f < 0.0 ? -1.0 : f + std::max(b, 0.0)};
        int cnt = 0;
        for (; cnt < kPhases && cnt < n; ++cnt) ms[cnt] = v[cnt];
        return cnt;
    }
    if (!h->shards.empty()) {
        int cnt = 0;
        for (size_t g = 0; g < h->shards.size(); ++g) {
            double cm[kPhases];
            cnt = grape_get_timings(h->shards[g], cm, n < kPhases ? n : kPhases);
            if (cnt < 0) return multi_fail(h, h->shards[g], cnt);
            for (int i = 0; i < cnt; ++i) ms[i] = g == 0 ? cm[i] : std::max(ms[i], cm[i]);
        }
        if (n > kPhases) { ms[kPhases] = h->host_enqueue_calls ? 2.0 * h->host_enqueue_ms / h->host_enqueue_calls : -1.0; cnt = kPhases + 1; }
        if (n > kPhases + 1) { ms[kPhases + 1] = (h->use_rccl && h->allreduce_calls) ? h->allreduce_ms / h->allreduce_calls : -1.0; cnt = kPhases + 2; }
        return cnt;
    }
    HIPCHK(h, hipSetDevice(h->device));
    HIPCHK(h, hipDeviceSynchronize());
    int cnt = 0;
    for (int i = 0; i < kPhases && i < n; ++i, ++cnt) {
        double sum = 0.0;
        int used = 0;
        for (int r = 0; r < kRing; ++r) {
            float t = 0.f;
            Phase &p = h->ph[r][i];
            if (p.used && hipEventElapsedTime(&t, p.e0, p.e1) == hipSuccess) { sum += t; ++used; }
        }
        ms[i] = used ? sum / used : -1.0;
    }
    return cnt;
}
GRAPE_BARRIER(h ? &h->err : &g_create_error)

int grape_reset_timings(grape_handle *h) try {
    if (!h) return GRAPE_ERR_INVALID;
    if (h->open) { h->open->ms_fwd = h->open->ms_bwd = 0.0; h->open->n_fwd = h->open->n_bwd = 0; return GRAPE_OK; }
    if (!h->shards.empty()) {
        for (grape_handle *c : h->shards) {
            const int rc = grape_reset_timings(c);
            if (rc) return multi_fail(h, c, rc);
        }
        h->host_enqueue_ms = 0.0;
        h->allreduce_ms = 0.0; h->allreduce_calls = 0;
        h->host_enqueue_calls = 0;
        return GRAPE_OK;
    }
    HIPCHK(h, hipSetDevice(h->device));
    HIPCHK(h, hipDeviceSynchronize());
    for (auto &ring : h->ph)
        for (auto &p : ring) p.used = false;
    h->n_fwd = h->n_bwd = 0;
    h->n_eval = 0;
    return GRAPE_OK;
}
GRAPE_BARRIER(h ? &h->err : &g_create_error)

int grape_get_work(grape_handle *h, double *out, int n) try {
    if (!h || !out || n < 4) return GRAPE_ERR_INVALID;
    if (h->open) return open_work(h, out, n);
    if (!h->shards.empty()) {
        const int m = n < 20 ? n : 20;
        std::fill(out, out + m, 0.0);
        for (grape_handle *c : h->shards) {
            double cw[20] = {0.};
            const int rc = grape_get_work(c, cw, m);
            if (rc < 0) return multi_fail(h, c, rc);
            for (int i = 0; i < m; ++i) out[i] = (i == 15 || i == 16 || i == 18) ? cw[i] : out[i] + cw[i];
        }
        if (m > 14 && out[14] > 0.0) out[14] = h->shards[0]->asm16p ? 3.0 : h->shards[0]->asm18gp ? 4.0 : h->shards[0]->asm18g ? 2.0 : 1.0;
        return 4;
    }
    HIPCHK(h, hipSetDevice(h->device));
    HIPCHK(h, hipDeviceSynchronize());
    if (h->credit_pending) {
        ExpmArgs ea{};
        ea.H0f = h->d_H0f; ea.Hcf = h->d_Hcf; ea.eps = h->d_eps; ea.shape = h->d_shape; ea.dts = h->d_dts;
        ea.flags = h->d_flags; ea.stats = h->d_stats; ea.Sf = h->d_Sf;
        ea.K = h->KC; ea.rep = h->d_rep; ea.L = h->L; ea.N_T = h->N_T; ea.hc_per_traj = h->p.hc_per_traj;
        ea.n1 = h->d_n1; ea.n1_k = h->K;
        HIPCHK(h, (hipError_t)grape_t16_credit_launch(&ea, sizeof(ea), (void *)h->stream));
        HIPCHK(h, hipStreamSynchronize(h->stream));
        h->credit_pending = false;
    }
    unsigned long long sh[GRAPE_STAT_SHARDS * GRAPE_STAT_SLOTS], st[GRAPE_STAT_SLOTS] = {0};
    HIPCHK(h, hipMemcpy(sh, h->d_stats, sizeof(sh), hipMemcpyDeviceToHost));
    for (int q = 0; q < GRAPE_STAT_SHARDS; ++q)
        for (int i = 0; i < GRAPE_STAT_SLOTS; ++i) st[i] += sh[q * GRAPE_STAT_SLOTS + i];
    const double N3 = (double)h->N * h->N * h->N, N2 = (double)h->N * h->N;
    const double cells = (double)h->K * h->N_T, ecells = (double)h->KC * h->N_T;
    const double gemms = 2.0 * st[3] + 3.0 * st[4] + 4.0 * st[5] + 5.0 * st[6] + 6.0 * st[7];
    out[0] = cells;
    out[1] = (double)st[0];
    out[2] = (gemms + (double)st[0]) * 8.0 * N3 + ecells * (32.0 / 3.0) * N3;
    out[3] = (double)st[8] * (1.0 + 2.0 * h->L) * 8.0 * N2;
    if (n > 4) out[4] = (double)st[8];
    if (n > 5) out[5] = (double)st[9];
    if (n > 6) out[6] = h->series ? 0.0 : ecells;
    if (n > 7) out[7] = (double)st[10];
    if (n > 8) out[8] = (double)st[11];
    if (n > 9) out[9] = (double)st[12] * 2048.0;
    if (n > 10) out[10] = (double)st[13];
    if (n > 11) out[11] = (double)st[14];
    if (n > 12) out[12] = h->u_fallback ? 1.0 : 0.0;
    if (n > 13) out[13] = (double)st[15];
    if (n > 14) out[14] = h->asm16p ? 3.0 : h->asm16 ? 1.0 : h->asm18gp ? 4.0 : h->asm18g ? 2.0 : 0.0;
    if (n > 15) {
        double kind = 0.0;
        if (!h->series && h->d_park3 && h->NT == 4) {
            if (h->deriv3_general) kind = 3.0;
            else if (h->L > 2) kind = 2.0;
            else if (!h->deriv3_h0g && h->deriv3_asm) kind = 1.0;
        } else if (!h->series && h->deriv4_blocks) kind = 4.0;
        out[15] = kind;
    }
    if (n > 16) out[16] = (h->large && !h->series && h->t18 && h->lg_asm) ? 1.0 : 0.0;
    if (n > 17) {
        double carried = 0.0;
        if (h->last_walk_fuse && h->d_prog) {
            std::vector<int> prog((size_t)2 * h->K);
            HIPCHK(h, hipMemcpy(prog.data(), h->d_prog, prog.size() * sizeof(int), hipMemcpyDeviceToHost));
            for (int k = 0; k < h->K; ++k) {
                if (h->last_walk_fuse & 1) carried += prog[(size_t)k];
                if (h->last_walk_fuse & 2) carried += prog[(size_t)h->K + k];
            }
        }
        out[17] = carried;
    }
    if (n > 18) out[18] = h->scan16 ? (double)h->scan_Bk : 0.0;
    if (n > 19) {
        double certified = 0.0;
        if (h->d_cert && h->d_splan && !h->series) {
            const size_t ncell = (size_t)h->KC * h->N_T;
            std::vector<int> plan(ncell);
            int fl[8];
            HIPCHK(h, hipMemcpy(plan.data(), h->d_splan, ncell * sizeof(int), hipMemcpyDeviceToHost));
            HIPCHK(h, hipMemcpy(fl, h->d_flags, sizeof(fl), hipMemcpyDeviceToHost));
            if (!(4L * fl[6] > (long)ncell))
                for (int w : plan) certified += (w & T16_PLAN_CERT) ? 1.0 : 0.0;
        }
        out[19] = certified;
    }
    return 4;
}
GRAPE_BARRIER(h ? &h->err : &g_create_error)

int grape_get_cert_table(grape_handle *h, int *dims, double *coef, int *exps) try {
    if (!h || !dims) return GRAPE_ERR_INVALID;
    if (h->open || !h->shards.empty()) {
        h->err = "grape_get_cert_table: a closed handle on one device";
        return GRAPE_ERR_INVALID;
    }
    const int nt = h->cert_n8 + h->cert_n6;
    dims[0] = h->KC; dims[1] = h->cert_n8; dims[2] = h->cert_n6;
    if (!h->d_cert || !nt) { dims[1] = dims[2] = 0; return GRAPE_OK; }
    HIPCHK(h, hipSetDevice(h->device));
    if (coef) HIPCHK(h, hipMemcpy(coef, h->d_cert, (size_t)h->KC * nt * sizeof(double), hipMemcpyDeviceToHost));
    if (exps) HIPCHK(h, hipMemcpy(exps, h->d_cert_exp, (size_t)nt * sizeof(int), hipMemcpyDeviceToHost));
    return GRAPE_OK;
}
GRAPE_BARRIER(h ? &h->err : &g_create_error)

int grape_get_time_gradient(grape_handle *h, double *dJdt) try {
    if (h && h->open) return open_refuse(h, "grape_get_time_gradient");
    if (!h || !dJdt) return GRAPE_ERR_INVALID;
    const int N_T = h->N_T;
    if (!h->shards.empty()) {
        std::vector<double> part((size_t)N_T);
        for (size_t g = 0; g < h->shards.size(); ++g) {
            const int rc = grape_get_time_gradient(h->shards[g], g == 0 ? dJdt : part.data());
            if (rc) return multi_fail(h, h->shards[g], rc);
            if (g > 0) for (int n = 0; n < N_T; ++n) dJdt[n] += part[n];
        }
        return GRAPE_OK;
    }
    if (h->tg_state != 3) {
        h->err = h->tg_state == 0 ? "grape_get_time_gradient: no complete gradient evaluation on this time grid (none yet, the last "
                                    "one failed, or grape_set_tlist came after it)"
               : h->tg_state == 1 ? "grape_get_time_gradient: the last evaluation had no gradient (grape_eval with G == NULL)"
                                  : "grape_get_time_gradient called between grape_forward and the backward half";
        return GRAPE_ERR_INVALID;
    }
    HIPCHK(h, hipSetDevice(h->device));
    if (h->foreign_stream) HIPCHK(h, hipDeviceSynchronize());
    (void)hipGetLastError();
    if (!h->d_tq) HIPCHK(h, h->mem.alloc(&h->d_tq, (size_t)h->K * N_T));
    if (!h->d_dJdt) HIPCHK(h, h->mem.alloc(&h->d_dJdt, (size_t)N_T));
    TimeGradArgs ta{};
    ta.H0f = h->d_H0f; ta.Hcf = h->d_Hcf; ta.eps = h->d_eps; ta.shape = h->d_shape;
    ta.fw = h->d_fw; ta.bw = h->d_bw; ta.rho = h->d_rho; ta.z = h->tg_unit ? h->d_z : nullptr;
    ta.gb = (h->have_gb && !h->tg_xi_user) ? h->d_gb : nullptr; ta.lambda_q = 0.25 * h->p.lambda_b;
    ta.out = h->d_tq;
    ta.K = h->K; ta.L = h->L; ta.N = h->N; ta.NP = h->NP; ta.N_T = N_T; ta.hc_per_traj = h->p.hc_per_traj;
    const int nct = h->NP <= 64 ? 4 : h->NP <= 128 ? 2 : 1;
    const size_t lds = (size_t)2 * h->NP * 16 * nct * sizeof(double);
    const dim3 grid((unsigned)((N_T + 16 * nct - 1) / (16 * nct)), (unsigned)h->K);
    int dev = 0;
    HIPCHK(h, hipGetDevice(&dev));
    static LdsLimit lim1, lim2, lim4;
    if (nct == 4) {
        HIPCHK(h, lim4.ensure((const void *)time_grad_kernel<4>, dev, lds));
        hipLaunchKernelGGL(time_grad_kernel<4>, grid, dim3(256), lds, h->stream, ta);
    } else if (nct == 2) {
        HIPCHK(h, lim2.ensure((const void *)time_grad_kernel<2>, dev, lds));
        hipLaunchKernelGGL(time_grad_kernel<2>, grid, dim3(256), lds, h->stream, ta);
    } else {
        HIPCHK(h, lim1.ensure((const void *)time_grad_kernel<1>, dev, lds));
        hipLaunchKernelGGL(time_grad_kernel<1>, grid, dim3(256), lds, h->stream, ta);
    }
    HIPCHK(h, hipGetLastError());
    hipLaunchKernelGGL(grad_reduce_kernel, dim3((N_T + 15) / 16), dim3(256), 0, h->stream, h->d_tq, h->K, N_T, h->d_dJdt,
                       (const double2 *)nullptr);
    HIPCHK(h, hipGetLastError());
    HIPCHK(h, hipMemcpyAsync(dJdt, h->d_dJdt, (size_t)N_T * 8, hipMemcpyDeviceToHost, h->stream));
    HIPCHK(h, hipStreamSynchronize(h->stream));
    return GRAPE_OK;
}
GRAPE_BARRIER(h ? &h->err : &g_create_error)

int grape_open_time_gradient(grape_handle *h, double *dJdt) try {
    if (!h) { g_create_error = "grape_open_time_gradient: h == NULL"; return GRAPE_ERR_INVALID; }
    if (!dJdt) { h->err = "grape_open_time_gradient: dJdt == NULL"; return GRAPE_ERR_INVALID; }
    if (!h->open) {
        h->err = "grape_open_time_gradient: not an open-system handle (grape_create_open); grape_get_time_gradient is the call for a closed one";
// ... 751 lines not shown
```

### grape.jl_amd/csrc/grape_kernels.hip.h

```cpp
#pragma once
#include <hip/hip_runtime.h>
#include <stdint.h>

#include "grape_t18_coeffs.h"

typedef double d4 __attribute__((ext_vector_type(4)));

#define MFMA64(a, b, c) __builtin_amdgcn_mfma_f64_16x16x4f64((a), (b), (c), 0, 0, 0)

__device__ __constant__ double c_pade3[4] = {120., 60., 12., 1.};
__device__ __constant__ double c_pade5[6] = {30240., 15120., 3360., 420., 30., 1.};
__device__ __constant__ double c_pade7[8] = {17297280., 8648640., 1995840., 277200., 25200., 1512., 56., 1.};
__device__ __constant__ double c_pade9[10] = {17643225600., 8821612800., 2075673600., 302702400.,
                                              30270240., 2162160., 110880., 3960., 90., 1.};
#define B13_0 64764752532480000.
#define B13_1 32382376266240000.
#define B13_2 7771770303897600.
#define B13_3 1187353796428800.
#define B13_4 129060195264000.
#define B13_5 10559470521600.
#define B13_6 670442572800.
#define B13_7 33522128640.
#define B13_8 1323241920.
#define B13_9 40840800.
#define B13_10 960960.
#define B13_11 16380.
#define B13_12 182.
#define B13_13 1.

#define GRAPE_STAT_SHARDS 64
#define GRAPE_STAT_SLOTS 16
__device__ __forceinline__ void stat_add(unsigned long long *stats, int idx, unsigned long long v) {
    atomicAdd(&stats[(size_t)(blockIdx.x & (GRAPE_STAT_SHARDS - 1)) * GRAPE_STAT_SLOTS + idx], v);
}

struct ExpmArgs {
    const double *H0f;
    const double *Hcf;
    const double *eps;
    const double *shape;
    const double *dts;
    double2 *U;
    int *flags;
    unsigned long long *stats;
    int K, L, N_T, hc_per_traj;
    const int *rep;
    int *cellflag;
    const double *n1;
    int n1_k;
    int *cell_list;
    int listed;
    const double *Sf;
#ifdef GRAPE_DIAG
    int ablate;
    unsigned long long *stamps;
#endif
};

#define T16_PLAN_R 1.15
#define T16_PLAN_RS 1.11
#define T16_PLAN_SMAX 3
struct T16PlanArgs {
    const double *gram;
    const double *eps, *shape, *dts;
    int *flags;
    int KC, L, N_T, N;
    int *splan;
    int sq_on;
    const double *cert;
    const int *cert_exp;
    int n8, n6;
    int *verdict;
};
#define T16_PLAN_SQ_MASK 0xFF
#define T16_PLAN_CERT 0x100
__device__ __forceinline__ bool t16_certified(const double *t, const int *ex, const int n8, const int n6, const int L, const double *e,
                                              const double dt, const int sq) {
    double p[2] = {0., 0.}, S8 = 0.;
    for (int i = 0; i < n8 + n6; ++i) {
        unsigned x = (unsigned)ex[i];
        double mono = 1.0;
        for (int l = 0; l < L; ++l, x >>= 4)
            for (unsigned q = x & 15u; q > 0; --q) mono *= e[l];
        const double c = t[i];
        p[i < n8 ? 0 : 1] += c * mono;
        if (i < n8) S8 += fabs(c) * fabs(mono);
    }
    const double dt2 = dt * dt, dt8 = (dt2 * dt2) * (dt2 * dt2);
    constexpr double th2 = T16_THETA * T16_THETA, th8 = (th2 * th2) * (th2 * th2);
    const double lhs = (p[0] + 0x1p-30 * S8) * dt8 * (1.0 + 1e-6), rhs = ldexp(th8, 8 * sq);
    return lhs <= rhs && p[1] >= 0.0;
}
__global__ void __launch_bounds__(256) t16_plan_kernel(T16PlanArgs a) {
    const int cell = blockIdx.x * 256 + threadIdx.x;
    bool out = false;
    if (cell < a.KC * a.N_T) {
        const int kc = cell / a.N_T, n = cell - kc * a.N_T, M = a.L + 1;
        const double *G = a.gram + (size_t)kc * (M * M + M), *kap = G + M * M;
        double e[9];
        e[0] = 1.0;
        for (int l = 0; l < a.L; ++l) e[1 + l] = a.eps[(size_t)l * a.N_T + n] * (a.shape ? a.shape[(size_t)l * a.N_T + n] : 1.0);
        double m2 = 0., wk = 0., w = 0.;
        for (int i = 0; i < M; ++i) {
            for (int j = 0; j < M; ++j) m2 += e[i] * e[j] * G[i * M + j];
            const double wi = fabs(e[i]) * sqrt(fmax(G[i * M + i], 0.0));
            w += wi; wk += wi * kap[i];
        }
        const double dt = a.dts[n];
        const double r = 2.0 * fabs(dt) * sqrt(fmax(m2, 0.0) / (double)a.N) * (w > 0.0 ? wk / w : 1.0);
        out = !(r <= T16_PLAN_R);
        if (a.splan) {
            int sq = 0;
            if (out && a.sq_on) {
                double rs = r;
                while (sq < T16_PLAN_SMAX && !(rs <= T16_PLAN_RS)) { rs *= 0.5; ++sq; }
                out = !(rs <= T16_PLAN_RS);
                if (out) sq = 0;
            }
            const bool cert = a.cert && t16_certified(a.cert + (size_t)kc * (a.n8 + a.n6), a.cert_exp, a.n8, a.n6, a.L, e + 1, dt, sq);
            if (cert) a.verdict[cell] = 0;
            a.splan[cell] = sq | (cert ? T16_PLAN_CERT : 0);
        }
    }
    const unsigned long long m = __ballot(out);
    if ((threadIdx.x & 63) == 0 && m) atomicAdd(&a.flags[6], (int)__popcll(m));
}
__device__ __forceinline__ bool t16_skipped(const int *flags, const int ncell) { return 4L * flags[6] > (long)ncell; }

struct CtrlSumArgs {
    const double *Hcf, *eps, *shape;
    double *Sf;
    int L, N_T, pp2;
    int per_traj;
    const int *rep;
};
__device__ __forceinline__ void ctrl_sum_body(CtrlSumArgs a) {
    const int blk = blockIdx.x, kc = a.per_traj ? blk / a.N_T : 0, n = blk - kc * a.N_T;
    if (a.per_traj) a.Hcf += (size_t)(a.rep ? a.rep[kc] : kc) * a.L * a.pp2;
    double e[8];
    for (int l = 0; l < a.L; ++l) e[l] = a.eps[(size_t)l * a.N_T + n] * (a.shape ? a.shape[(size_t)l * a.N_T + n] : 1.0);
    double2 *dst = (double2 *)(a.Sf + (size_t)blk * a.pp2);
#pragma unroll 4
    for (int i = blockIdx.y * blockDim.x + threadIdx.x; i < a.pp2 / 2; i += gridDim.y * blockDim.x) {
        double2 acc = make_double2(0., 0.);
        for (int l = 0; l < a.L; ++l) {
            const double2 h = ((const double2 *)(a.Hcf + (size_t)l * a.pp2))[i];
            acc.x = fma(e[l], h.x, acc.x); acc.y = fma(e[l], h.y, acc.y);
        }
        dst[i] = acc;
    }
}
__global__ void __launch_bounds__(256) ctrl_sum_kernel(CtrlSumArgs a) { ctrl_sum_body(a); }

__global__ void __launch_bounds__(256) dte_kernel(const double *eps, const double *shape, const double *dts, int L, int N_T, int slots, double *out) {
    const int n = blockIdx.x * blockDim.x + threadIdx.x;
    if (n >= N_T) return;
    double *row = out + (size_t)2 * slots * n;
    row[0] = dts[n];
    for (int l = 0; l < 2 * slots - 1; ++l)
        row[1 + l] = l < L ? eps[(size_t)l * N_T + n] * (shape ? shape[(size_t)l * N_T + n] : 1.0) : 0.0;
}

template <int NT>
struct Strip {
    d4 re[NT];
    d4 im[NT];
};

template <int NT>
__device__ __forceinline__ void strip_zero(Strip<NT> &s) {
#pragma unroll
    for (int t = 0; t < NT; ++t) {
        s.re[t] = (d4){0., 0., 0., 0.};
        s.im[t] = (d4){0., 0., 0., 0.};
    }
}

template <int NT>
struct Strip3 {
    d4 p1[NT], p2[NT], p3[NT];
};
template <int NT>
__device__ __forceinline__ void strip3_zero(Strip3<NT> &q) {
#pragma unroll
    for (int t = 0; t < NT; ++t) { q.p1[t] = (d4){0., 0., 0., 0.}; q.p2[t] = (d4){0., 0., 0., 0.}; q.p3[t] = (d4){0., 0., 0., 0.}; }
}
template <int NT>
__device__ __forceinline__ void strip3_add_to(const Strip3<NT> &q, Strip<NT> &acc) {
#pragma unroll
    for (int t = 0; t < NT; ++t) {
        acc.re[t] += q.p1[t] - q.p2[t];
        acc.im[t] += q.p3[t] - q.p1[t] - q.p2[t];
    }
}

template <int NT, int LD>
__device__ __forceinline__ void gemm_xb3(Strip3<NT> &q, const double *__restrict__ Xre,
                                         const double *__restrict__ Xim, const Strip<NT> &B, int lane) {
    const double *__restrict__ xr = Xre + (lane & 15) * LD + (lane >> 4);
    const double *__restrict__ xi = Xim + (lane & 15) * LD + (lane >> 4);
    double are[NT], aim[NT];
#pragma unroll
    for (int tr = 0; tr < NT; ++tr) {
        are[tr] = xr[16 * tr * LD];
        aim[tr] = xi[16 * tr * LD];
    }
#pragma unroll
    for (int t = 0; t < NT; ++t) {
#pragma unroll
        for (int r = 0; r < 4; ++r) {
            const int ks = 4 * t + r;
            const double bre = B.re[t][r], bim = B.im[t][r];
            const double bs = bre + bim;
            double as[NT];
#pragma unroll
            for (int tr = 0; tr < NT; ++tr) as[tr] = are[tr] + aim[tr];
#pragma unroll
            for (int tr = 0; tr < NT; ++tr) q.p1[tr] = MFMA64(are[tr], bre, q.p1[tr]);
            __builtin_amdgcn_sched_barrier(0);
            if (ks + 1 < 4 * NT) {
#pragma unroll
                for (int tr = 0; tr < NT; ++tr) are[tr] = xr[16 * tr * LD + 4 * (ks + 1)];
            }
            __builtin_amdgcn_sched_barrier(0);
#pragma unroll
            for (int tr = 0; tr < NT; ++tr) q.p2[tr] = MFMA64(aim[tr], bim, q.p2[tr]);
            __builtin_amdgcn_sched_barrier(0);
            if (ks + 1 < 4 * NT) {
#pragma unroll
                for (int tr = 0; tr < NT; ++tr) aim[tr] = xi[16 * tr * LD + 4 * (ks + 1)];
            }
            __builtin_amdgcn_sched_barrier(0);
#pragma unroll
            for (int tr = 0; tr < NT; ++tr) q.p3[tr] = MFMA64(as[tr], bs, q.p3[tr]);
// ... 1592 lines not shown
        STAMP(4);
        st_s += s; st_max = max(st_max, s);
        st_ord[order == 13 ? 4 : (order - 3) / 2] += 1;
        if (s > 0) __syncthreads();
    }
#ifdef GRAPE_DIAG
    if (tid0 == 0) g_diag_off[blockIdx.x & 1023] = 0;
#endif
    if (tid0 == 0) {
        stat_add(a.stats, 0, (unsigned long long)st_s);
#pragma unroll
        for (int o = 0; o < 5; ++o)
            if (st_ord[o]) stat_add(a.stats, 3 + o, (unsigned long long)st_ord[o]);
        if (st_max > 0) atomicMax(&a.flags[1], st_max);
    }
}

template <int NT, bool HERM>
__global__ void __launch_bounds__(NT * 64) expm_persistent_kernel(ExpmArgs a) {
    expm_persistent<NT, HERM>(a, threadIdx.x);
}

template <int NT, bool PIVOTED, bool HERM = false>
__global__ void __launch_bounds__(NT * 64) expm_pade_kernel(ExpmArgs a) {
    const int ncell = a.K * a.N_T;
    if constexpr (!PIVOTED) {
        expm_single<NT, HERM>(a, xcd_remap(blockIdx.x, ncell), threadIdx.x);
    } else {
        if (a.flags[2] == 0) return;
        for (int cell = blockIdx.x; cell < ncell; cell += gridDim.x) {
            if (!a.cellflag[cell]) continue;
            __syncthreads();
            expm_cell_pivoted<NT>(a, cell);
        }
    }
}

struct SweepArgs {
    const double2 *U;
    const double2 *psi0;
    const double2 *target;
    const double *weights;
    double2 *store;
    double2 *tau;
    const double *f;
    double *rho;
    int *flags;
    double chi_min_norm;
    int K, K_total, N, N_T, functional;
    const int *cls;
    const double2 *xi;
    const double *wq;
    double lambda_b;
    const double *inv_tnorm;
    int unit_chi;
    const double2 *chi_in;
    int drop_sibling;
    const int *resume;
    int *xcc;
};

__device__ __forceinline__ void chi_coefficient(const SweepArgs &a, const int k, double &cr, double &ci) {
    if (a.unit_chi) { cr = a.inv_tnorm[k]; ci = 0.; return; }
    const double w = a.weights ? a.weights[k] : 1.0;
    const double Kt = (double)a.K_total;
    if (a.functional == 0) { cr = w * a.f[0] / (Kt * Kt); ci = w * a.f[1] / (Kt * Kt); }
    else if (a.functional == 1) { const double2 t = a.tau[k]; cr = w * t.x / Kt; ci = w * t.y / Kt; }
    else { cr = w / (2.0 * Kt); ci = 0.; }
}

__device__ __forceinline__ double2 chi_boundary(const SweepArgs &a, const int k, const int i) {
    if (a.chi_in) return a.chi_in[(size_t)k * a.N + i];
    double cr, ci;
    chi_coefficient(a, k, cr, ci);
    const double2 t = a.target[(size_t)k * a.N + i];
    return make_double2(cr * t.x - ci * t.y, cr * t.y + ci * t.x);
}

struct ChiCoeffArgs {
    SweepArgs s;
    double *rho;
    double2 *z;
};
__device__ __forceinline__ void chi_coeff_body(const ChiCoeffArgs &a) {
    const int k = blockIdx.x * blockDim.x + threadIdx.x;
    if (k >= a.s.K) return;
    SweepArgs s = a.s;
    s.unit_chi = 0;
    double cr, ci;
    chi_coefficient(s, k, cr, ci);
    const double tn = 1.0 / a.s.inv_tnorm[k];
    const double rho = sqrt(cr * cr + ci * ci) * tn;
    a.rho[k] = rho;
    a.z[k] = make_double2(cr * tn, -ci * tn);
    if (rho < a.s.chi_min_norm) atomicOr(&a.s.flags[0], 2);
}
__global__ void chi_coeff_kernel(ChiCoeffArgs a) { chi_coeff_body(a); }

__device__ __forceinline__ double wave_sum(double v) {
#pragma unroll
    for (int off = 32; off >= 1; off >>= 1) v += __shfl_xor(v, off, 64);
    return v;
}

template <int H, int OFF, int RWT>
__device__ __forceinline__ void rs_step(double (&pr)[RWT], double (&pi)[RWT], int lane, int &row) {
    const bool up = (lane & OFF) != 0;
#pragma unroll
    for (int r = 0; r < H; ++r) {
        const double sr = up ? pr[r] : pr[r + H], si = up ? pi[r] : pi[r + H];
        const double kr = up ? pr[r + H] : pr[r], ki = up ? pi[r + H] : pi[r];
        pr[r] = kr + __shfl_xor(sr, OFF, 64);
        pi[r] = ki + __shfl_xor(si, OFF, 64);
    }
    row += up ? H : 0;
}

template <int NP, bool BACKWARD>
__device__ __forceinline__ void sweep_body(const SweepArgs &a, const int k) {
    constexpr int NW = NP == 48 ? 3 : 4, RW = NP / NW;
    __shared__ double2 x[2][NP];
    __shared__ double2 part[NW][NP];
    __shared__ double sc[4];
    const int tid = threadIdx.x, lane = tid & 63, wave = tid >> 6;
    const double2 *Uk = a.U + (size_t)(a.cls ? a.cls[k] : k) * a.N_T * NP * NP;
    double2 *st = a.store + (size_t)k * (a.N_T + 1) * NP;

    if (!BACKWARD) {
        if (tid < NP) {
            double2 v = tid < a.N ? a.psi0[(size_t)k * a.N + tid] : make_double2(0., 0.);
            x[0][tid] = v;
            st[tid] = v;
        }
    } else {
        double2 v = make_double2(0., 0.);
        if (tid < a.N) {
            v = chi_boundary(a, k, tid);
            if (a.xi) {
                const double2 x_ = a.xi[((size_t)k * (a.N_T + 1) + a.N_T) * NP + tid];
                const double c = a.lambda_b * a.wq[a.N_T];
                v.x += c * x_.x; v.y += c * x_.y;
            }
        }
        if (wave == 0) {
            double n2 = wave_sum(lane < NP ? v.x * v.x + v.y * v.y : 0.);
            if (lane == 0) sc[0] = sqrt(n2);
        }
        __syncthreads();
        const double rho = sc[0];
        if (tid == 0 && !a.unit_chi) {
            a.rho[k] = rho;
            if (rho < a.chi_min_norm) atomicOr(&a.flags[0], 2);
        }
        if (tid < NP) {
            const double ir = rho > 0. ? 1.0 / rho : 0.;
            v.x *= ir; v.y *= ir;
            x[0][tid] = v;
            st[(size_t)a.N_T * NP + tid] = v;
        }
    }
    __syncthreads();
    const int step_start = a.resume ? min(max(a.resume[k], 0), a.N_T) : 0;
    if (step_start > 0) {
        if (tid < NP) x[0][tid] = st[(size_t)(BACKWARD ? a.N_T - step_start : step_start) * NP + tid];
        __syncthreads();
    }

    int cur = 0;
    auto load_tile = [&](double2 (&dst)[RW], int step) __attribute__((always_inline)) {
        const int nn = BACKWARD ? a.N_T - 1 - step : step;
        const double2 *Un = Uk + (size_t)nn * NP * NP;
#pragma unroll
        for (int r = 0; r < RW; ++r)
            {
                typedef double v2d __attribute__((ext_vector_type(2)));
                const v2d t = lane < NP ? __builtin_nontemporal_load((const v2d *)&Un[(size_t)(wave * RW + r) * NP + lane]) : (v2d){0., 0.};
                dst[r] = make_double2(t.x, t.y);
// ... 890 lines not shown
                for (int l = 0; l < LMAX; ++l) {
                    pwr += e[l] * mur[l];
                    pwi += e[l] * mui[l];
                    phr[l] += sh[l] * mur[l];
                    phi[l] += sh[l] * mui[l];
                }
#pragma unroll
                for (int r = 0; r < 4; ++r) {
                    const size_t o = (size_t)(16 * rt + 4 * r + rg) * 16 + c;
                    vn[0 * vplane + o] = pwr[r];
                    vn[1 * vplane + o] = pwi[r];
                }
#pragma unroll
                for (int l = 0; l < LMAX; ++l) {
                    double orr = 0., oi = 0., nn = 0.;
#pragma unroll
                    for (int r = 0; r < 4; ++r) {
                        const size_t o = (size_t)(16 * rt + 4 * r + rg) * 16 + c;
                        vn[((1 + l) * 2 + 0) * vplane + o] = phr[l][r];
                        vn[((1 + l) * 2 + 1) * vplane + o] = phi[l][r];
                        orr += phr[l][r] * psr[tt][r] + phi[l][r] * psi_[tt][r];
                        oi += phr[l][r] * psi_[tt][r] - phi[l][r] * psr[tt][r];
                        nn += phr[l][r] * phr[l][r] + phi[l][r] * phi[l][r];
                    }
                    orr += __shfl_xor(orr, 16, 64); oi += __shfl_xor(oi, 16, 64); nn += __shfl_xor(nn, 16, 64);
                    orr += __shfl_xor(orr, 32, 64); oi += __shfl_xor(oi, 32, 64); nn += __shfl_xor(nn, 32, 64);
                    sor[l] += orr; soi[l] += oi; snn[l] += nn;
                }
            }
            if (lane < 16) {
#pragma unroll
                for (int l = 0; l < LMAX; ++l) {
                    red[slot][wave][l][c][0] = sor[l];
                    red[slot][wave][l][c][1] = soi[l];
                    red[slot][wave][l][c][2] = snn[l];
                }
            }
            __syncthreads();
            const double al2 = alr * alr + ali * ali;
#pragma unroll
            for (int l = 0; l < LMAX; ++l) {
                if (l < L && !((done_mask >> l) & 1)) {
                    double orr = 0., oi = 0., nn = 0.;
#pragma unroll
                    for (int w = 0; w < NW; ++w) {
                        orr += red[slot][w][l][c][0]; oi += red[slot][w][l][c][1]; nn += red[slot][w][l][c][2];
                    }
                    accr[l] += alr * orr + ali * oi;
                    acci[l] += alr * oi - ali * orr;
                    if (m >= 2 && al2 * nn < a.tol * a.tol) done_mask |= 1 << l;
                }
            }
            cur ^= 1;
            if (__all(done_mask == all_done)) { converged = 1; m_used = m; break; }
            {
                const double f = dt / (double)(m + 1);
                const double nr = -ali * f, ni = alr * f;
                alr = nr; ali = ni;
            }
        }
        if (tid < 16 && valid) {
            for (int l = 0; l < L; ++l) {
                double gr_ = 0., gi_ = 0.;
#pragma unroll
                for (int ll = 0; ll < LMAX; ++ll) if (ll == l) { gr_ = accr[ll]; gi_ = acci[ll]; }
                a.tg[((size_t)k * L + l) * a.N_T + n] = make_double2(rho * gr_, rho * gi_);
            }
        }
        if (tid == 0) {
            const bool redone = a.batch_flag && a.batch_flag[batch];
            if (!converged && !redone) atomicOr(&a.flags[0], 4);
            if (!redone) stat_add(a.stats, 8, (unsigned long long)m_used * (unsigned long long)min(16, a.N_T - n0));
        }
        __syncthreads();
    }
}

struct DerivFlagArgs {
    const double *rb, *eps, *shape, *dts;
    int rb_k, K, L, N_T, hc_per_traj, batches_per_k, nbatch_total;
    double sub_theta;
    int *batch_flag, *flags;
};
__global__ void deriv_flag_kernel(DerivFlagArgs a) {
    const int batch = blockIdx.x * blockDim.x + threadIdx.x;
    if (batch >= a.nbatch_total) return;
    const int k = batch / a.batches_per_k, n0 = (batch - k * a.batches_per_k) * 16;
    int ns = 1;
    for (int n = n0; n < min(n0 + 16, a.N_T); ++n)
        ns = max(ns, deriv_substeps(a.rb, a.rb_k, a.sub_theta, k, a.hc_per_traj, a.L, a.eps, a.shape, a.N_T, n, a.dts[n]));
    a.batch_flag[batch] = ns > 1;
    if (ns > 1) atomicAdd(&a.flags[3], 1);
}

struct DerivEconArgs {
    const int *verdict, *splan, *cls, *flags;
    const int *cell_deg;
    int K, KC, N_T, batches_per_k, nbatch_total;
    int deg0, deg1;
    int *batch_econ;
};
__global__ void deriv_econ_kernel(DerivEconArgs a) {
    const int batch = blockIdx.x * blockDim.x + threadIdx.x;
    if (batch >= a.nbatch_total) return;
    const int k = batch / a.batches_per_k, n0 = (batch - k * a.batches_per_k) * 16;
    const int kc = a.cls ? a.cls[k] : k;
    bool ok = a.cell_deg || !t16_skipped(a.flags, a.KC * a.N_T);
    int deg = 0;
    for (int n = n0; ok && n < min(n0 + 16, a.N_T); ++n) {
        const int cell = kc * a.N_T + n;
        int d;
        if (a.cell_deg) d = a.cell_deg[cell];
        else {
            const int sq = a.splan ? (a.splan[cell] & T16_PLAN_SQ_MASK) : 0;
            d = a.verdict[cell] != 0 ? 0 : sq == 0 ? a.deg0 : sq == 1 ? a.deg1 : 0;
        }
        ok = d > 0;
        deg = max(deg, d);
    }
    a.batch_econ[batch] = ok ? deg : 0;
}

struct DerivSubArgs {
    DerivMfmaArgs m;
    const double *rb;
    int rb_k;
    double sub_theta;
    const int *batch_flag;
};

template <int NP, int LMAX>
__global__ void __launch_bounds__((NP / 16 <= 8 ? NP / 16 : 8) * 64) deriv_sub_kernel(DerivSubArgs b) {
    const DerivMfmaArgs &a = b.m;
    constexpr int RT = NP / 16, KS = NP / 4;
    constexpr int NW = RT <= 8 ? RT : 8, TPW = RT / NW, NV = 1 + LMAX;
    static_assert(RT % NW == 0, "row tiles must divide evenly over the waves");
    __shared__ double red[2][NW][NV][16];
    __shared__ double redo[NW][LMAX][16][2];
    if (b.batch_flag && a.flags[3] == 0) return;
    const int tid = threadIdx.x, lane = tid & 63;
    const int wave = __builtin_amdgcn_readfirstlane(tid >> 6);
    const int c = lane & 15, rg = lane >> 4;
    const int L = a.L;
    const size_t vplane = (size_t)NP * 16;
    double *vbase = a.vecs + (size_t)blockIdx.x * 2 * NV * 2 * vplane;
    for (int batch = blockIdx.x; batch < a.nbatch_total; batch += gridDim.x) {
        if (b.batch_flag && !b.batch_flag[batch]) continue;
        const int k = batch / a.batches_per_k;
        const int n0 = (batch - k * a.batches_per_k) * 16;
        const int n = n0 + c;
        const bool valid = n < a.N_T;
        const int nc = valid ? n : a.N_T - 1;
        const double *h0k = a.H0p + (size_t)k * RT * KS * 128;
        const double *hck = a.Hcp + (size_t)(a.hc_per_traj ? k : 0) * L * RT * KS * 128;
        const double dt = a.dts[nc];
        double e[LMAX], sh[LMAX];
#pragma unroll
        for (int l = 0; l < LMAX; ++l) {
            sh[l] = (l < L && a.shape) ? a.shape[(size_t)l * a.N_T + nc] : 1.0;
            e[l] = l < L ? a.eps[(size_t)l * a.N_T + nc] * sh[l] : 0.;
        }
        int nsub = valid ? deriv_substeps(b.rb, b.rb_k, b.sub_theta, k, a.hc_per_traj, L, a.eps, a.shape, a.N_T, nc, dt) : 1;
#pragma unroll
        for (int off = 1; off < 16; off <<= 1) nsub = max(nsub, __shfl_xor(nsub, off, 64));
        nsub = __builtin_amdgcn_readfirstlane(nsub);
        const double dts_ = dt / (double)nsub;
        const double rho = a.rho[k];
        double psr[TPW][4], psi_[TPW][4];
        d4 chr[TPW], chi_[TPW], gfr[LMAX][TPW], gfi[LMAX][TPW];
#pragma unroll
        for (int tt = 0; tt < TPW; ++tt) {
#pragma unroll
            for (int r = 0; r < 4; ++r) {
                const int row = 16 * (wave + tt * NW) + 4 * r + rg;
                const double2 p = a.fw[((size_t)k * (a.N_T + 1) + nc) * NP + row];
                const double2 x = a.bw[((size_t)k * (a.N_T + 1) + nc + 1) * NP + row];
                psr[tt][r] = p.x; psi_[tt][r] = p.y;
                chr[tt][r] = valid ? x.x : 0.; chi_[tt][r] = valid ? x.y : 0.;
            }
#pragma unroll
            for (int l = 0; l < LMAX; ++l) { gfr[l][tt] = (d4){0., 0., 0., 0.}; gfi[l][tt] = (d4){0., 0., 0., 0.}; }
        }
        const int all_done = ((1 << L) - 1) | (1 << LMAX);
        int converged = 1;
        unsigned long long orders = 0;
        for (int sub = 0; sub < nsub; ++sub) {
            __syncthreads();
#pragma unroll
            for (int tt = 0; tt < TPW; ++tt)
#pragma unroll
                for (int r = 0; r < 4; ++r) {
                    const size_t o = (size_t)(16 * (wave + tt * NW) + 4 * r + rg) * 16 + c;
                    vbase[0 * vplane + o] = chr[tt][r];
                    vbase[1 * vplane + o] = chi_[tt][r];
#pragma unroll
                    for (int l = 0; l < LMAX; ++l) {
                        vbase[((1 + l) * 2 + 0) * vplane + o] = gfr[l][tt][r];
                        vbase[((1 + l) * 2 + 1) * vplane + o] = gfi[l][tt][r];
                    }
                }
            __syncthreads();
            d4 ocr[TPW], oci[TPW];
#pragma unroll
// ... 504 lines not shown
            if (!converged && !redone) atomicOr(&a.flags[0], 4);
            if (!redone) stat_add(a.stats, 8, (unsigned long long)M * (unsigned long long)min(16, a.N_T - n0));
        }
        __syncthreads();
    }
}

struct GbArgs {
    const double2 *Dt;
    const double2 *fw;
    double2 *xi;
    double *gb;
    int NP, N_T, d_per_traj;
};
__global__ void __launch_bounds__(256) gb_kernel(GbArgs a) {
    __shared__ double2 psi[512];
    __shared__ double part[256];
    const int NP = a.NP, tid = threadIdx.x;
    const int cell = blockIdx.x;
    const int k = cell / (a.N_T + 1);
    const double2 *Dt = a.Dt + (size_t)(a.d_per_traj ? k : 0) * NP * NP;
    for (int i = tid; i < NP; i += 256) psi[i] = a.fw[(size_t)cell * NP + i];
    __syncthreads();
    double acc = 0.;
    for (int i = tid; i < NP; i += 256) {
        double ar = 0., ai = 0.;
        for (int j = 0; j < NP; ++j) {
            const double2 d = Dt[(size_t)j * NP + i], p = psi[j];
            ar += d.x * p.x - d.y * p.y;
            ai += d.x * p.y + d.y * p.x;
        }
        a.xi[(size_t)cell * NP + i] = make_double2(-ar, -ai);
        acc += psi[i].x * ar + psi[i].y * ai;
    }
    part[tid] = acc;
    __syncthreads();
    for (int off = 128; off >= 1; off >>= 1) {
        if (tid < off) part[tid] += part[tid + off];
        __syncthreads();
    }
    if (tid == 0) a.gb[cell] = part[0];
}
__global__ void __launch_bounds__(256) jb_reduce_kernel(const double *gb, const double *wq, int K, int N_T, double *out) {
    __shared__ double part[256];
    double s = 0.;
    const size_t tot = (size_t)K * (N_T + 1);
    for (size_t i = threadIdx.x; i < tot; i += 256) s += wq[i % (N_T + 1)] * gb[i];
    part[threadIdx.x] = s;
    __syncthreads();
    for (int off = 128; off >= 1; off >>= 1) {
        if (threadIdx.x < off) part[threadIdx.x] += part[threadIdx.x + off];
        __syncthreads();
    }
    if (threadIdx.x == 0) out[0] = part[0];
}

__device__ __forceinline__ void grad_reduce_body(double2 *tg, int K, int LN, double *G, const double2 *z) {
    __shared__ double part[16][17];
    const int j = threadIdx.x & 15, kg = threadIdx.x >> 4;
    const int idx = blockIdx.x * 16 + j;
    double s = 0.;
    if (idx < LN) {
        if (z) {
            for (int k = kg; k < K; k += 16) {
                const double2 t = tg[(size_t)k * LN + idx], zk = z[k];
                const double2 v = make_double2(zk.x * t.x - zk.y * t.y, zk.x * t.y + zk.y * t.x);
                tg[(size_t)k * LN + idx] = v;
                s += v.x;
            }
        } else {
            for (int k = kg; k < K; k += 16) s += tg[(size_t)k * LN + idx].x;
        }
    }
    part[kg][j] = s;
    __syncthreads();
    if (kg == 0 && idx < LN) {
        double t = 0.;
#pragma unroll
        for (int q = 0; q < 16; ++q) t += part[q][j];
        G[idx] = -2.0 * t;
    }
}
__global__ void __launch_bounds__(256) grad_reduce_kernel(double2 *tg, int K, int LN, double *G, const double2 *z) { grad_reduce_body(tg, K, LN, G, z); }
```

### grape.jl_amd/csrc/grape_t18.hip

```cpp
#include <hip/hip_runtime.h>
#include <stdint.h>
#include <string.h>
#include <type_traits>
#include <mutex>
#include <vector>
#include <stdlib.h>
#include <stdio.h>
namespace {
#include "grape_t18.hip.h"
#define GRAPE_BATCH_T18_UNIT
#include "grape_batch.hip.h"
#include "grape_deriv3.hip.h"
#include "grape_econ_coeffs.h"

template <int NT, bool SYM, bool CHEB, bool T16 = false>
hipError_t launch(const ExpmArgs &a, hipStream_t s, int blocks) {
    static size_t lds_set[64] = {0};
    const size_t lds = sizeof(double) * (size_t)T18Lds<NT>::TOTAL;
    int dev = 0;
    hipGetDevice(&dev);
    if (lds_set[dev & 63] < lds) {
        hipError_t e = hipFuncSetAttribute((const void *)expm_t18_kernel<NT, SYM, CHEB, T16>, hipFuncAttributeMaxDynamicSharedMemorySize, (int)lds);
        if (e != hipSuccess) return e;
        lds_set[dev & 63] = lds;
// ... 52 lines not shown
        if (skip_if_flagged || a.d.gpark) return (int)hipErrorInvalidValue;
        return (int)launch_d3_asm(a, s, blocks);
    }
    if (NT == 4 && L <= 2) {
        if (asm_ok && !skip_if_flagged && !a.d.gpark) return (int)launch_d3_asm(a, s, blocks);
        return (int)(L == 1 ? launch_d3<4, 1>(a, s, blocks) : launch_d3<4, 2>(a, s, blocks));
    }
    return (int)hipErrorInvalidValue;
}

extern "C" const unsigned char grape_asm_co_start[], grape_asm_co_end[];
namespace {
struct T16AsmArgs {
    const double *H0f, *Sf, *dts;
    double2 *U;
    int *verdict;
    const int *rep;
    int KC, N_T, nblk;
    int fuse;
    unsigned long long *diag;
    const int *flags;
    const int *wgtab;
    const double2 *xinit;
    double2 *fw, *bw;
    int *prog;
    int K, s_per_cell;
    const int *splan;
};
static_assert(sizeof(T16AsmArgs) == 136, "argument block of the assembly kernel");

__device__ __forceinline__ double t16_post_norm1(const ExpmArgs &a, const int cell, double *red, const int tid) {
    constexpr int NP = 64;
    const int kc = cell / a.N_T, n = cell - kc * a.N_T, k = a.rep ? a.rep[kc] : kc;
    const double *h0 = a.H0f + (size_t)k * 2 * NP * NP, *sn = a.Sf + (size_t)(a.hc_per_traj ? cell : n) * 2 * NP * NP;
    const double dt = a.dts[n];
    const int j = tid & 63, part = tid >> 6;
    double sum = 0.;
    for (int i = part; i < NP; i += 4) {
        const double xr = dt * (h0[NP * NP + i * NP + j] + sn[NP * NP + i * NP + j]), xi = -dt * (h0[i * NP + j] + sn[i * NP + j]);
        sum += fast_sqrt(xr * xr + xi * xi);
    }
    red[tid] = sum;
    __syncthreads();
    if (tid < 64) {
        double c = red[tid] + red[64 + tid] + red[128 + tid] + red[192 + tid];
#pragma unroll
        for (int off = 32; off >= 1; off >>= 1) c = fmax(c, __shfl_xor(c, off, 64));
        if (tid == 0) red[256] = c;
    }
    __syncthreads();
    const double nA = red[256];
    __syncthreads();
    return nA;
}

__global__ void __launch_bounds__(256) t16_post_kernel(ExpmArgs a, const int *verdict, const int *prog, int nprog, const int *splan) {
    const int tid = threadIdx.x, lane = tid & 63, ncell = a.K * a.N_T;
    if (t16_skipped(a.flags, ncell)) return;
    if (prog && blockIdx.x == 0) {
        unsigned long long steps = 0;
        for (int i = tid; i < nprog; i += 256) steps += (unsigned long long)prog[i];
        for (int off = 32; off >= 1; off >>= 1) steps += __shfl_xor(steps, off, 64);
        if (lane == 0 && steps) stat_add(a.stats, 12, steps * 4ull * 2ull);
    }
    const int cell = blockIdx.x * 256 + tid;
    const bool valid = cell < ncell;
    const bool ok = valid && verdict[cell] == 0;
    if (valid && !ok) a.cell_list[atomicAdd(&a.flags[4], 1)] = cell;
    const unsigned long long m_ok = __ballot(ok), m_valid = __ballot(valid);
    {
        unsigned long long sq = valid ? (unsigned long long)(splan[cell] & T16_PLAN_SQ_MASK) : 0ull;
        unsigned long long sq_ok = ok ? sq : 0ull;
        for (int off = 32; off >= 1; off >>= 1) { sq += __shfl_xor(sq, off, 64); sq_ok += __shfl_xor(sq_ok, off, 64); }
        if (lane == 0 && sq) stat_add(a.stats, 12, sq * 4ull * 192ull);
        if (lane == 0 && sq_ok) stat_add(a.stats, 13, sq_ok);
    }
    if (lane == 0 && m_valid) {
        stat_add(a.stats, 12, (unsigned long long)__popcll(m_valid) * 4ull * (unsigned long long)(T16Count<4>::CELL + 1));
        if (m_ok) {
            stat_add(a.stats, 14, (unsigned long long)__popcll(m_ok));
            stat_add(a.stats, 15, (unsigned long long)__popcll(m_ok));
        }
        atomicAdd(&a.flags[5], (int)__popcll(m_valid));
    }
}

__global__ void __launch_bounds__(256) t16_credit_kernel(ExpmArgs a) {
    __shared__ double red[264];
    __shared__ int todo[256], ntodo;
    __shared__ unsigned long long cnt[8];
    const int tid = threadIdx.x, lane = tid & 63, ncell = a.K * a.N_T;
    if (t16_skipped(a.flags, ncell)) return;
    if (tid < 8) cnt[tid] = 0;
    if (tid == 0) ntodo = 0;
    __syncthreads();
    auto order_of = [](double nA) { return nA > 2.1 ? 4 : nA > 0.95 ? 3 : nA > 0.25 ? 2 : nA > 0.015 ? 1 : 0; };
    auto squarings_of = [](double nA) {
        if (!(nA > 5.4)) return 0;
        const double r = nA / 5.4;
        const int e = ilogb(r);
        return (r == ldexp(1.0, e)) ? e : e + 1;
    };
    const int cell = blockIdx.x * 256 + tid;
    bool cert = false;
    if (cell < ncell) {
        const double bound = expm_norm_bound(a, cell);
        cert = bound > 2.1 && bound <= 5.4;
        if (!cert) todo[atomicAdd(&ntodo, 1)] = cell;
    }
    const unsigned long long m_cert = __ballot(cert);
    if (lane == 0 && m_cert) atomicAdd(&cnt[2 + 4], (unsigned long long)__popcll(m_cert));
    __syncthreads();
    const int nt = ntodo;
    for (int q = 0; q < nt; ++q) {
        const double nA = t16_post_norm1(a, todo[q], red, tid);
        if (tid == 0) {
            const int sj = squarings_of(nA);
            if (sj) { cnt[0] += (unsigned long long)sj; cnt[1] = max(cnt[1], (unsigned long long)sj); }
            cnt[2 + order_of(nA)] += 1ull;
        }
    }
    __syncthreads();
    if (tid == 0) {
        if (cnt[0]) stat_add(a.stats, 0, cnt[0]);
        for (int o = 0; o < 5; ++o)
            if (cnt[2 + o]) stat_add(a.stats, 3 + o, cnt[2 + o]);
        if (cnt[1]) atomicMax(&a.flags[1], (int)cnt[1]);
    }
}

constexpr int D3_INV_TABLE = 2048;
constexpr int D3_PAIRS_OFF = 32768, D3_ECON_OFF = 32768, D3_ECON_TAB_B = 512;
struct AsmModule {
    hipModule_t mod = nullptr;
    hipFunction_t fn = nullptr, fn_d3 = nullptr, fn_d3s = nullptr, fn_lg = nullptr, fn_d3g = nullptr, fn_d4[2] = {nullptr, nullptr};
    hipFunction_t fn_t18g = nullptr, fn_t16p = nullptr, fn_t16p4 = nullptr, fn_t18gp = nullptr;
    double *inv = nullptr;
};
hipError_t asm_function(int dev, hipFunction_t *fn, hipFunction_t *fn_d3 = nullptr, const double **inv = nullptr,
                        hipFunction_t *fn_d3s = nullptr, hipFunction_t *fn_lg = nullptr, hipFunction_t *fn_d3g = nullptr,
                        hipFunction_t *fn_d4 = nullptr, int d4_index = 0, hipFunction_t *fn_t18g = nullptr,
                        hipFunction_t *fn_t16p = nullptr, int t16p_slots = 2) {
    static AsmModule mods[64];
    static std::mutex mtx;
    std::lock_guard<std::mutex> lock(mtx);
    AsmModule &m = mods[dev & 63];
    if (!m.fn) {
        static std::vector<char> override_co;
        const void *image = (const void *)grape_asm_co_start;
        if (const char *path = getenv("GRAPE_ASM_CO")) {
            if (override_co.empty()) {
                if (FILE *f = fopen(path, "rb")) {
                    fseek(f, 0, SEEK_END);
                    const long n = ftell(f);
                    fseek(f, 0, SEEK_SET);
                    if (n > 0) {
                        override_co.resize((size_t)n);
                        if (fread(override_co.data(), 1, (size_t)n, f) != (size_t)n) override_co.clear();
                    }
                    fclose(f);
                }
            }
            if (override_co.empty()) return hipErrorFileNotFound;
            image = override_co.data();
        }
        hipError_t e = hipModuleLoadData(&m.mod, image);
// ... 102 lines not shown
extern "C" const double *grape_econ_pairs(void) {
    int dev = 0;
    if (hipGetDevice(&dev) != hipSuccess) return nullptr;
    hipFunction_t fn;
    const double *inv = nullptr;
    if (asm_function(dev, nullptr, &fn, &inv) != hipSuccess || !inv) return nullptr;
    static_assert(D3_ECON_TAB_B == 64 * 8, "64 doubles per degree");
    return inv + (D3_PAIRS_OFF + D3_ECON_OFF) / 8;
}

namespace {
struct D4AsmArgs {
    const double *H0q, *Hcq, *H0p, *Hcp, *eps, *shape, *dts;
    const double2 *fw, *bw;
    const double *rho;
    double2 *tg;
    double *park;
    int *flags;
    unsigned long long *stats;
    const int *batch_flag;
    const double *inv;
    int K, L, N_T, hc_per_traj, nbatch_total, batches_per_k, mcap, slots;
    double tol2;
    int deep, nblocks;
};
static_assert(sizeof(D4AsmArgs) == 176, "argument block of the assembly kernel");
}
extern "C" int grape_deriv4_launch(int NP, const void *d2args, size_t d2size, const double *H0q3, const double *Hcq3, const double *H0p3,
                                   const double *Hcp3, void *stream, int blocks) {
    if (d2size != sizeof(Deriv2Args) || (NP != 128 && NP != 256) || blocks < 1) return (int)hipErrorInvalidValue;
    Deriv2Args a;
    memcpy(&a, d2args, sizeof(a));
    if (a.L < 1 || a.L > 8 || a.gpark || a.maxm + 2 > D3_INV_TABLE || !H0q3 || !Hcq3 || !H0p3 || !Hcp3) return (int)hipErrorInvalidValue;
    if ((long)a.N_T + 1 >= (1L << 19) || (long)a.K * a.L * a.N_T >= (1L << 27) || a.nbatch_total >= (1 << 24)) return (int)hipErrorInvalidValue;
    int dev = 0;
    hipError_t e = hipGetDevice(&dev);
    if (e != hipSuccess) return (int)e;
    hipFunction_t fn;
    const double *inv;
    e = asm_function(dev, nullptr, nullptr, &inv, nullptr, nullptr, nullptr, &fn, NP == 256);
    if (e != hipSuccess) return (int)e;
    D4AsmArgs k{};
    k.H0q = H0q3; k.Hcq = Hcq3; k.H0p = H0p3; k.Hcp = Hcp3; k.eps = a.eps; k.shape = a.shape; k.dts = a.dts; k.fw = a.fw; k.bw = a.bw;
    k.rho = a.rho; k.tg = a.tg; k.park = a.park; k.flags = a.flags; k.stats = a.stats; k.batch_flag = a.batch_flag; k.inv = inv;
    k.K = a.K; k.L = a.L; k.N_T = a.N_T; k.hc_per_traj = a.hc_per_traj; k.nbatch_total = a.nbatch_total; k.batches_per_k = a.batches_per_k;
    k.mcap = a.max_order < a.maxm ? a.max_order : a.maxm;
    k.slots = a.maxm + 1;
    k.tol2 = a.tol * a.tol;
    k.deep = (a.batch_econ && a.batch_flag && k.mcap >= ECON_MAXDEG) ? 2 : 0;
    k.nblocks = blocks;
    size_t size = sizeof(k);
    void *cfg[] = {HIP_LAUNCH_PARAM_BUFFER_POINTER, &k, HIP_LAUNCH_PARAM_BUFFER_SIZE, &size, HIP_LAUNCH_PARAM_END};
    return (int)hipModuleLaunchKernel(fn, (unsigned)blocks, 1, 1, 256, 1, 1, 0, (hipStream_t)stream, nullptr, cfg);
}

extern "C" int grape_lg_asm_launch(const void *k, size_t size, unsigned blocks, void *stream) {
    if (size != 416 || blocks == 0) return (int)hipErrorInvalidValue;
    int dev = 0;
    hipError_t e = hipGetDevice(&dev);
    if (e != hipSuccess) return (int)e;
    hipFunction_t fn;
    e = asm_function(dev, nullptr, nullptr, nullptr, nullptr, &fn);
    if (e != hipSuccess) return (int)e;
    unsigned char buf[416];
    memcpy(buf, k, sizeof(buf));
    size_t sz = sizeof(buf);
    void *cfg[] = {HIP_LAUNCH_PARAM_BUFFER_POINTER, buf, HIP_LAUNCH_PARAM_BUFFER_SIZE, &sz, HIP_LAUNCH_PARAM_END};
    return (int)hipModuleLaunchKernel(fn, blocks, 1, 1, 256, 1, 1, 0, (hipStream_t)stream, nullptr, cfg);
}

extern "C" void grape_t16_walks(int KC, int N_T, int nblk, int *tab) {
    const long ncell = (long)KC * N_T;
    for (int b = 0; b < nblk; ++b) {
        const long lo = b * ncell / nblk, hi = (b + 1) * ncell / nblk;
        int *e = tab + 4 * b;
        e[3] = 0;
        if (hi == lo) { e[0] = 0; e[1] = 0; e[2] = 1; }
        else if (lo % N_T == 0 || hi % N_T != 0) { e[0] = (int)lo; e[1] = (int)(hi - lo); e[2] = 1; }
        else { e[0] = (int)(hi - 1); e[1] = (int)(hi - lo); e[2] = -1; }
    }
}

extern "C" int grape_t16_asm_launch(const void *args, size_t args_size, int *verdict, void *stream, int blocks,
                                    const void *const *walk, int fuse, int K) {
    if (args_size != sizeof(ExpmArgs)) return (int)hipErrorInvalidValue;
    ExpmArgs a;
    memcpy(&a, args, sizeof(a));
    if (!a.Sf || !verdict || blocks < 1 || !walk || !walk[0] || !walk[5]) return (int)hipErrorInvalidValue;
    if (fuse && (!walk[1] || !walk[2] || !walk[3] || !walk[4] || a.rep || K != a.K)) return (int)hipErrorInvalidValue;
    const long ncell = (long)a.K * a.N_T;
    if (ncell <= 0 || ncell >= (1L << 28)) return (int)hipErrorInvalidValue;
    int dev = 0;
    hipError_t e = hipGetDevice(&dev);
    if (e != hipSuccess) return (int)e;
    hipFunction_t fn;
    e = asm_function(dev, &fn);
    if (e != hipSuccess) return (int)e;
    T16AsmArgs k{};
    k.H0f = a.H0f; k.Sf = a.Sf; k.dts = a.dts; k.U = a.U; k.verdict = verdict; k.rep = a.rep;
    k.KC = a.K; k.N_T = a.N_T; k.nblk = blocks; k.flags = a.flags;
    k.fuse = fuse; k.wgtab = (const int *)walk[0]; k.xinit = (const double2 *)walk[1]; k.fw = (double2 *)walk[2];
    k.bw = (double2 *)walk[3]; k.prog = (int *)walk[4]; k.K = K; k.splan = (const int *)walk[5];
    k.s_per_cell = a.hc_per_traj ? 1 : 0;
    size_t size = sizeof(k);
    void *cfg[] = {HIP_LAUNCH_PARAM_BUFFER_POINTER, &k, HIP_LAUNCH_PARAM_BUFFER_SIZE, &size, HIP_LAUNCH_PARAM_END};
    hipStream_t s = (hipStream_t)stream;
    e = hipModuleLaunchKernel(fn, (unsigned)blocks, 1, 1, 256, 1, 1, 0, s, nullptr, cfg);
    if (e != hipSuccess) return (int)e;
    hipLaunchKernelGGL(t16_post_kernel, dim3((unsigned)((ncell + 255) / 256)), dim3(256), 0, s, a, (const int *)verdict,
                       fuse ? (const int *)walk[4] : (const int *)nullptr, 2 * K, (const int *)walk[5]);
    return (int)hipGetLastError();
}

extern "C" int grape_t16p_asm_launch(const void *args, size_t args_size, int *verdict, void *stream, int blocks,
                                     const void *const *walk, int fuse, int K, const double *dte) {
    if (args_size != sizeof(ExpmArgs)) return (int)hipErrorInvalidValue;
    ExpmArgs a;
    memcpy(&a, args, sizeof(a));
    if (!a.hc_per_traj || a.L < 1 || a.L > 4 || !dte || !verdict || blocks < 1 || !walk || !walk[0] || !walk[5]) return (int)hipErrorInvalidValue;
    if (fuse && (!walk[1] || !walk[2] || !walk[3] || !walk[4] || a.rep || K != a.K)) return (int)hipErrorInvalidValue;
    const long ncell = (long)a.K * a.N_T;
    if (ncell <= 0 || ncell >= (1L << 28)) return (int)hipErrorInvalidValue;
    int dev = 0;
    hipError_t e = hipGetDevice(&dev);
    if (e != hipSuccess) return (int)e;
    hipFunction_t fn;
    e = asm_function(dev, nullptr, nullptr, nullptr, nullptr, nullptr, nullptr, nullptr, 0, nullptr, &fn, a.L <= 2 ? 2 : 4);
    if (e != hipSuccess) return (int)e;
    T16AsmArgs k{};
    k.H0f = a.H0f; k.Sf = a.Hcf; k.dts = dte; k.U = a.U; k.verdict = verdict; k.rep = a.rep;
    k.KC = a.K; k.N_T = a.N_T; k.nblk = blocks; k.flags = a.flags;
    k.fuse = fuse; k.wgtab = (const int *)walk[0]; k.xinit = (const double2 *)walk[1]; k.fw = (double2 *)walk[2];
    k.bw = (double2 *)walk[3]; k.prog = (int *)walk[4]; k.K = K; k.splan = (const int *)walk[5];
    k.s_per_cell = a.L;
    size_t size = sizeof(k);
    void *cfg[] = {HIP_LAUNCH_PARAM_BUFFER_POINTER, &k, HIP_LAUNCH_PARAM_BUFFER_SIZE, &size, HIP_LAUNCH_PARAM_END};
    hipStream_t s = (hipStream_t)stream;
    e = hipModuleLaunchKernel(fn, (unsigned)blocks, 1, 1, 256, 1, 1, 0, s, nullptr, cfg);
    if (e != hipSuccess) return (int)e;
    hipLaunchKernelGGL(t16_post_kernel, dim3((unsigned)((ncell + 255) / 256)), dim3(256), 0, s, a, (const int *)verdict,
                       fuse ? (const int *)walk[4] : (const int *)nullptr, 2 * K, (const int *)walk[5]);
    return (int)hipGetLastError();
}

namespace {
__global__ void __launch_bounds__(256) t18g_post_kernel(ExpmArgs a, const int *verdict, const int *prog, int nprog, const int *splan) {
    const int tid = threadIdx.x, lane = tid & 63, ncell = a.K * a.N_T;
    if (prog && blockIdx.x == 0) {
        unsigned long long steps = 0;
        for (int i = tid; i < nprog; i += 256) steps += (unsigned long long)prog[i];
        for (int off = 32; off >= 1; off >>= 1) steps += __shfl_xor(steps, off, 64);
        if (lane == 0 && steps) stat_add(a.stats, 12, steps * 4ull * 2ull);
    }
    const int cell = blockIdx.x * 256 + tid;
    const bool valid = cell < ncell;
    const bool bad = valid && verdict[cell] != 0;
    unsigned long long sq = valid ? (unsigned long long)splan[cell] : 0ull;
    for (int off = 32; off >= 1; off >>= 1) sq += __shfl_xor(sq, off, 64);
    const unsigned long long m_valid = __ballot(valid), m_bad = __ballot(bad);
    if (lane == 0 && m_valid) {
        const unsigned long long nc = (unsigned long long)__popcll(m_valid);
        stat_add(a.stats, 12, 4ull * (nc * (5ull * 192ull + 2ull) + sq * 192ull));
        if (sq) stat_add(a.stats, 13, sq);
        stat_add(a.stats, 14, nc);
        if (m_bad) atomicOr(&a.flags[0], 64);
    }
}
}

extern "C" int grape_t18g_asm_launch(const void *args, size_t args_size, int *verdict, void *stream, int blocks,
                                     const void *const *walk, int fuse, int K, const double *dte) {
    if (args_size != sizeof(ExpmArgs)) return (int)hipErrorInvalidValue;
    ExpmArgs a;
    memcpy(&a, args, sizeof(a));
    if ((!a.Sf && !dte) || !verdict || blocks < 1 || !walk || !walk[0] || !walk[5]) return (int)hipErrorInvalidValue;
    if (dte && (!a.hc_per_traj || a.L < 1 || a.L > 2)) return (int)hipErrorInvalidValue;
    if (fuse && (!walk[1] || !walk[2] || !walk[3] || !walk[4] || a.rep || K != a.K)) return (int)hipErrorInvalidValue;
    const long ncell = (long)a.K * a.N_T;
    if (ncell <= 0 || ncell >= (1L << 28)) return (int)hipErrorInvalidValue;
    int dev = 0;
    hipError_t e = hipGetDevice(&dev);
    if (e != hipSuccess) return (int)e;
    hipFunction_t fn;
    if (dte) e = asm_function(dev, nullptr, nullptr, nullptr, nullptr, nullptr, nullptr, nullptr, 0, nullptr, &fn, 0);
    else e = asm_function(dev, nullptr, nullptr, nullptr, nullptr, nullptr, nullptr, nullptr, 0, &fn);
    if (e != hipSuccess) return (int)e;
    T16AsmArgs k{};
    k.H0f = a.H0f; k.Sf = dte ? a.Hcf : a.Sf; k.dts = dte ? dte : a.dts; k.U = a.U; k.verdict = verdict; k.rep = a.rep;
    k.KC = a.K; k.N_T = a.N_T; k.nblk = blocks; k.flags = a.flags;
    k.fuse = fuse; k.wgtab = (const int *)walk[0]; k.xinit = (const double2 *)walk[1]; k.fw = (double2 *)walk[2];
    k.bw = (double2 *)walk[3]; k.prog = (int *)walk[4]; k.K = K; k.splan = (const int *)walk[5];
// ... 61 lines not shown
```

Measured before the change: 54.80.

## Chain eval prologue, post/econ, and chi-coeff into fewer fused launches

Adds an eval-chain mode, on by default when the asm16 path is used. The control sum, t16 plan (with monomial tables in LDS), deriv flag, prog memset and chi-coeff work are folded into one prologue kernel, and the post-processing is merged with econ classification. The chi-coefficient computation moves into the gradient reduce kernel. This cuts the number of small kernel launches and memsets per gradient evaluation, at the cost of more complex fused kernels and redundant per-block chi computation in the reduce.

```diff
diff --git a/grape.jl_amd/api.py b/grape.jl_amd/api.py
--- a/grape.jl_amd/api.py
+++ b/grape.jl_amd/api.py
@@ -490,13 +490,13 @@
         self._chk(self._lib.grape_reset_timings(self._h))
 
     def work(self):
-        w = np.zeros(20)
-        self._lib.grape_get_work(self._h, w.ctypes.data, 20)
+        w = np.zeros(21)
+        self._lib.grape_get_work(self._h, w.ctypes.data, 21)
         return dict(cells=w[0], squarings=w[1], flop_expm=w[2], flop_deriv=w[3], deriv_orders=w[4],
                     pivoted_cells=w[5], expm_cells=w[6], series_terms=w[7], series_steps=w[8],
                     t18_mfma_flop=w[9], t18_squarings=w[10], t18_cells=w[11], matrix_free_fallback=w[12], t16_cells=w[13],
                     asm_kernel=w[14], asm_deriv_kernel=w[15], asm_blocked_products=w[16],
-                    walk_steps=w[17], scan_block=w[18], t16_certified=w[19])
+                    walk_steps=w[17], scan_block=w[18], t16_certified=w[19], deriv_sub_batches=w[20])
 
     def cert_table(self):
         dims = np.zeros(3, np.int32)
diff --git a/grape.jl_amd/csrc/grape_hip.hip b/grape.jl_amd/csrc/grape_hip.hip
--- a/grape.jl_amd/csrc/grape_hip.hip
+++ b/grape.jl_amd/csrc/grape_hip.hip
@@ -121,6 +121,7 @@
     int asm_blocks = 0;
     int last_walk_fuse = 0;
     bool asm_sq = true;
+    bool eval_chain = false;
     int asm_walk = 0;
     bool foreign_stream = false;
     bool credit_pending = false;
@@ -327,7 +328,7 @@
 extern "C" int grape_t18g_asm_launch(const void *args, size_t args_size, int *verdict, void *stream, int blocks,
                                      const void *const *walk, int fuse, int K, const double *dte);
 extern "C" int grape_t16_asm_launch(const void *args, size_t args_size, int *verdict, void *stream, int blocks,
-                                    const void *const *walk, int fuse, int K);
+                                    const void *const *walk, int fuse, int K, int chain, const void *econ, size_t econ_size);
 extern "C" int grape_t18_batch_launch(int herm, const void *args, size_t args_size, const void *strides, size_t strides_size,
                                       int sets, void *stream, int blocks);
 extern "C" void grape_t16_walks(int KC, int N_T, int nblk, int *tab);
@@ -1272,6 +1273,16 @@
 thread_local const std::vector<double> *tl_forced_bal = nullptr;
 int multi_fail(grape_handle *h, grape_handle *c, int rc);
 int backward_device_impl(grape_handle *h, const double *d_f, double *d_G, hipStream_t s, const double2 *d_chi);
+DerivEconArgs deriv_econ_args(const grape_handle *h) {
+    DerivEconArgs ec{};
+    ec.verdict = h->d_cellflag; ec.splan = h->d_splan; ec.cls = h->d_cls; ec.flags = h->d_flags;
+    ec.cell_deg = h->large ? h->d_celldeg : nullptr;
+    ec.deg0 = ECON_DEG[0]; ec.deg1 = ECON_DEG[ECON_NSETS - 1];
+    static_assert(ECON_NSETS == 4, "segments 1.36 (verdict), 1.6, 2.0 (blocked path), 2.72 (one planned squaring)");
+    ec.K = h->K; ec.KC = h->KC; ec.N_T = h->N_T; ec.batches_per_k = (h->N_T + 15) / 16;
+    ec.nbatch_total = h->K * ec.batches_per_k; ec.batch_econ = h->d_batchflag + ec.nbatch_total;
+    return ec;
+}
 double open_lambda_b(const grape_handle *h);
 
 double functional_from_sums(const grape_handle *h, const double *sums) {
@@ -2570,6 +2581,10 @@
     h->asm16p = h->asm16 && p_direct;
     h->asm18gp = h->asm18g && p_direct;
     {
+        const char *envch = getenv("GRAPE_EVAL_CHAIN");
+        h->eval_chain = h->asm16 && !h->asm16p && !(envch && atoi(envch) == 0);
+    }
+    {
         const char *enve = getenv("GRAPE_DERIV_ECON");
         const bool lg_ok = h->large && h->t18 && h->herm && !h->series;
         const bool t16c_ok = h->t16 && h->t18 && h->herm && !h->large && !h->series && (h->NT >= 3 || (h->NT == 2 && h->t18_small));
@@ -2806,6 +2821,7 @@
 #endif
     hipError_t e = hipSuccess;
     int walk_fuse = 0;
+    bool econ_chained = false;
     if (!h->series) {
         phase_begin(h, 0, s);
         if (h->large) {
@@ -2815,6 +2831,39 @@
             const int per_cu = h->NT == 1 ? 10 : h->NT == 2 ? 4 : 1;
             const int t18_blocks = 8 * (int)std::max<long>(1, std::min<long>((long)(h->num_cus / 8) * per_cu, (ncell + 7) / 8));
             if (h->t18 && (h->NT >= 3 || h->t18_small)) {
+                const int walk16 = h->asm_walk & (1 | ((h->fuse && h->fuse_on && h->want_bw) ? 2 : 0));
+                const bool chain = h->eval_chain && h->d_Sf && h->d_celllist;
+                if (chain) {
+                    EvalPrologueArgs pa{};
+                    CtrlSumArgs &ca = pa.cs;
+                    ca.Hcf = h->d_Hcf; ca.eps = h->d_eps; ca.shape = h->d_shape; ca.Sf = h->d_Sf;
+                    ca.L = h->L; ca.N_T = h->N_T; ca.pp2 = 2 * h->NP * h->NP;
+                    ca.per_traj = h->p.hc_per_traj ? 1 : 0; ca.rep = h->d_rep;
+                    pa.sum_x = (ca.per_traj ? h->KC : 1) * h->N_T; pa.sum_parts = std::max(1, ca.pp2 / 2 / 2048);
+                    T16PlanArgs &pl = pa.pl;
+                    pl.gram = h->d_gram; pl.eps = h->d_eps; pl.shape = h->d_shape; pl.dts = h->d_dts; pl.flags = h->d_flags;
+                    pl.KC = h->KC; pl.L = h->L; pl.N_T = h->N_T; pl.N = h->N;
+                    pl.splan = (h->asm_sq || h->d_cert) ? h->d_splan : nullptr;
+                    pl.sq_on = h->asm_sq ? 1 : 0;
+                    static_assert(GRAPE_CERT_LMAX <= T16_PLAN_PW_LMAX, "the power table of the plan holds the controls of every trace table");
+                    pl.cert = h->d_cert; pl.cert_exp = h->d_cert_exp; pl.n8 = h->cert_n8; pl.n6 = h->cert_n6;
+                    pl.verdict = h->d_cellflag;
+                    pa.plan_blocks = h->N_T;
+                    if (h->sub_theta > 0.0) {
+                        DerivFlagArgs &fa = pa.fl;
+                        fa.rb = h->d_rb; fa.eps = h->d_eps; fa.shape = h->d_shape; fa.dts = h->d_dts;
+                        fa.rb_k = h->K; fa.K = h->K; fa.L = h->L; fa.N_T = h->N_T; fa.hc_per_traj = h->p.hc_per_traj;
+                        fa.batches_per_k = (h->N_T + 15) / 16; fa.nbatch_total = h->K * fa.batches_per_k;
+                        fa.sub_theta = h->sub_theta; fa.batch_flag = h->d_batchflag; fa.flags = h->d_flags;
+                        pa.flag_blocks = (fa.nbatch_total + 255) / 256;
+                    }
+                    if (walk16) { pa.prog = h->d_prog; pa.nprog = 2 * h->K; }
+                    const long nblk = (long)pa.sum_x * pa.sum_parts + pa.plan_blocks + pa.flag_blocks + 1;
+                    if (nblk >= (1L << 31)) { h->err = "too many cells for one prologue launch"; return GRAPE_ERR_INVALID; }
+                    hipLaunchKernelGGL(eval_prologue_kernel, dim3((unsigned)nblk), dim3(256), 0, s, pa);
+                    HIPCHK(h, hipGetLastError());
+                    ea.Sf = h->d_Sf;
+                } else
                 if (h->d_Sf) {
                     CtrlSumArgs ca{};
                     ca.Hcf = h->d_Hcf; ca.eps = h->d_eps; ca.shape = h->d_shape; ca.Sf = h->d_Sf;
@@ -2826,7 +2875,7 @@
                 }
                 const bool t16 = h->d_celllist != nullptr;
                 ea.cell_list = h->d_celllist; ea.listed = 0;
-                if (t16) {
+                if (t16 && !chain) {
                     T16PlanArgs pa{};
                     pa.gram = h->d_gram; pa.eps = h->d_eps; pa.shape = h->d_shape; pa.dts = h->d_dts; pa.flags = h->d_flags;
                     pa.KC = h->KC; pa.L = h->L; pa.N_T = h->N_T; pa.N = h->N;
@@ -2862,10 +2911,14 @@
                     e = (hipError_t)grape_t16p_asm_launch(&ea, sizeof(ea), h->d_cellflag, (void *)s, h->asm_blocks, walk, walk_fuse, h->K, h->d_dte);
                 }
                 else if (t16 && h->asm16) {
-                    walk_fuse = h->asm_walk & (1 | ((h->fuse && h->fuse_on && h->want_bw) ? 2 : 0));
-                    if (walk_fuse) HIPCHK(h, hipMemsetAsync(h->d_prog, 0, (size_t)2 * h->K * sizeof(int), s));
+                    walk_fuse = walk16;
+                    if (walk_fuse && !chain) HIPCHK(h, hipMemsetAsync(h->d_prog, 0, (size_t)2 * h->K * sizeof(int), s));
                     const void *walk[6] = {h->d_wgtab, h->d_xinit, h->d_fw, h->d_bw, h->d_prog, h->d_splan};
-                    e = (hipError_t)grape_t16_asm_launch(&ea, sizeof(ea), h->d_cellflag, (void *)s, h->asm_blocks, walk, walk_fuse, h->K);
+                    DerivEconArgs ec{};
+                    econ_chained = chain && h->deriv_econ;
+                    if (econ_chained) ec = deriv_econ_args(h);
+                    e = (hipError_t)grape_t16_asm_launch(&ea, sizeof(ea), h->d_cellflag, (void *)s, h->asm_blocks, walk, walk_fuse, h->K,
+                                                         chain ? 1 : 0, econ_chained ? &ec : nullptr, sizeof(ec));
                     h->credit_pending = true;
                 }
                 else
@@ -2888,14 +2941,8 @@
             }
         }
         HIPCHK(h, e);
-        if (h->deriv_econ) {
-            DerivEconArgs ec{};
-            ec.verdict = h->d_cellflag; ec.splan = h->d_splan; ec.cls = h->d_cls; ec.flags = h->d_flags;
-            ec.cell_deg = h->large ? h->d_celldeg : nullptr;
-            ec.deg0 = ECON_DEG[0]; ec.deg1 = ECON_DEG[ECON_NSETS - 1];
-            static_assert(ECON_NSETS == 4, "segments 1.36 (verdict), 1.6, 2.0 (blocked path), 2.72 (one planned squaring)");
-            ec.K = h->K; ec.KC = h->KC; ec.N_T = h->N_T; ec.batches_per_k = (h->N_T + 15) / 16;
-            ec.nbatch_total = h->K * ec.batches_per_k; ec.batch_econ = h->d_batchflag + ec.nbatch_total;
+        if (h->deriv_econ && !econ_chained) {
+            const DerivEconArgs ec = deriv_econ_args(h);
             hipLaunchKernelGGL(deriv_econ_kernel, dim3((unsigned)((ec.nbatch_total + 255) / 256)), dim3(256), 0, s, ec);
             HIPCHK(h, hipGetLastError());
         }
@@ -3046,11 +3093,14 @@
     const bool unit = h->bw_done && !d_chi && !h->xi_user;
     h->bw_done = false;
     if (d_chi || h->xi_user) h->bw_unit = false;
+    ChiCoeffArgs cza{};
     if (unit) {
-        ChiCoeffArgs ca{};
-        ca.s = sa; ca.s.inv_tnorm = h->d_inv_tnorm; ca.rho = h->d_rho; ca.z = h->d_z;
-        hipLaunchKernelGGL(chi_coeff_kernel, dim3((h->K + 63) / 64), dim3(64), 0, s, ca);
-        e = hipGetLastError();
+        cza.s = sa; cza.s.inv_tnorm = h->d_inv_tnorm; cza.rho = h->d_rho; cza.z = h->d_z;
+        e = hipSuccess;
+        if (!h->eval_chain) {
+            hipLaunchKernelGGL(chi_coeff_kernel, dim3((h->K + 63) / 64), dim3(64), 0, s, cza);
+            e = hipGetLastError();
+        }
         h->z_valid = true;
     } else if (h->series && h->large) {
         e = launch_cheby(h, nullptr, &sa, s);
@@ -3088,7 +3138,7 @@
     da.cells_per_block = cpb;
     const int nblocks = h->K * ((h->N_T + cpb - 1) / cpb);
     phase_begin(h, 3, s);
-    if (h->NP >= 48 && h->sub_theta > 0.0) {
+    if (h->NP >= 48 && h->sub_theta > 0.0 && !h->eval_chain) {
         HIPCHK(h, hipMemsetAsync(h->d_flags + 3, 0, sizeof(int), s));
         DerivFlagArgs fa{};
         fa.rb = h->d_rb; fa.eps = h->d_eps; fa.shape = h->d_shape; fa.dts = h->d_dts;
@@ -3200,8 +3250,11 @@
     phase_end(h, 3, s);
     phase_begin(h, 4, s);
     const int LN = h->L * h->N_T;
-    hipLaunchKernelGGL(grad_reduce_kernel, dim3((LN + 15) / 16), dim3(256), 0, s, h->d_tg, h->K, LN, d_G,
-                       unit ? (const double2 *)h->d_z : (const double2 *)nullptr);
+    if (unit && h->eval_chain)
+        hipLaunchKernelGGL(grad_reduce_chi_kernel, dim3((LN + 15) / 16), dim3(256), 0, s, h->d_tg, h->K, LN, d_G, cza);
+    else
+        hipLaunchKernelGGL(grad_reduce_kernel, dim3((LN + 15) / 16), dim3(256), 0, s, h->d_tg, h->K, LN, d_G,
+                           unit ? (const double2 *)h->d_z : (const double2 *)nullptr);
     HIPCHK(h, hipGetLastError());
     phase_end(h, 4, s);
     if (!h->capturing) h->n_bwd++;
@@ -3910,10 +3963,10 @@
     if (!h || !out || n < 4) return GRAPE_ERR_INVALID;
     if (h->open) return open_work(h, out, n);
     if (!h->shards.empty()) {
-        const int m = n < 20 ? n : 20;
+        const int m = n < 21 ? n : 21;
         std::fill(out, out + m, 0.0);
         for (grape_handle *c : h->shards) {
-            double cw[20] = {0.};
+            double cw[21] = {0.};
             const int rc = grape_get_work(c, cw, m);
             if (rc < 0) return multi_fail(h, c, rc);
             for (int i = 0; i < m; ++i) out[i] = (i == 15 || i == 16 || i == 18) ? cw[i] : out[i] + cw[i];
@@ -3990,6 +4043,11 @@
                 for (int w : plan) certified += (w & T16_PLAN_CERT) ? 1.0 : 0.0;
         }
         out[19] = certified;
+    }
+    if (n > 20) {
+        int fl[8] = {0};
+        if (h->NP >= 48 && h->sub_theta > 0.0) HIPCHK(h, hipMemcpy(fl, h->d_flags, sizeof(fl), hipMemcpyDeviceToHost));
+        out[20] = (double)fl[3];
     }
     return 4;
 }
diff --git a/grape.jl_amd/csrc/grape_kernels.hip.h b/grape.jl_amd/csrc/grape_kernels.hip.h
--- a/grape.jl_amd/csrc/grape_kernels.hip.h
+++ b/grape.jl_amd/csrc/grape_kernels.hip.h
@@ -91,10 +91,43 @@
     const double lhs = (p[0] + 0x1p-30 * S8) * dt8 * (1.0 + 1e-6), rhs = ldexp(th8, 8 * sq);
     return lhs <= rhs && p[1] >= 0.0;
 }
-__global__ void __launch_bounds__(256) t16_plan_kernel(T16PlanArgs a) {
-    const int cell = blockIdx.x * 256 + threadIdx.x;
-    bool out = false;
-    if (cell < a.KC * a.N_T) {
+#define T16_PLAN_PW_LMAX 4
+#define T16_PLAN_MONO_MAX (495 + 210)
+__device__ __forceinline__ void t16_plan_monomials(const T16PlanArgs &a, const int n, double *lds) {
+    double *pw = lds, *mono = lds + 9 * T16_PLAN_PW_LMAX;
+    if ((int)threadIdx.x < a.L) {
+        const int l = threadIdx.x;
+        const double el = a.eps[(size_t)l * a.N_T + n] * (a.shape ? a.shape[(size_t)l * a.N_T + n] : 1.0);
+        double v = 1.0;
+        for (int q = 0; q <= 8; ++q, v *= el) pw[9 * l + q] = v;
+    }
+    __syncthreads();
+    for (int i = threadIdx.x; i < a.n8 + a.n6; i += blockDim.x) {
+        unsigned x = (unsigned)a.cert_exp[i];
+        double m = pw[min(x & 15u, 8u)];
+        for (int l = 1; l < a.L; ++l) { x >>= 4; m *= pw[9 * l + min(x & 15u, 8u)]; }
+        mono[i] = m;
+    }
+    __syncthreads();
+}
+__device__ __forceinline__ bool t16_certified_mono(const double *t, const double *mono, const int n8, const int n6, const double dt, const int sq) {
+    double p8 = 0., p6 = 0., S8 = 0.;
+#pragma unroll 8
+    for (int i = 0; i < n8; ++i) {
+        const double c = t[i], m = mono[i];
+        p8 += c * m;
+        S8 += fabs(c) * fabs(m);
+    }
+#pragma unroll 8
+    for (int i = n8; i < n8 + n6; ++i) p6 += t[i] * mono[i];
+    const double dt2 = dt * dt, dt8 = (dt2 * dt2) * (dt2 * dt2);
+    constexpr double th2 = T16_THETA * T16_THETA, th8 = (th2 * th2) * (th2 * th2);
+    const double lhs = (p8 + 0x1p-30 * S8) * dt8 * (1.0 + 1e-6), rhs = ldexp(th8, 8 * sq);
+    return lhs <= rhs && p6 >= 0.0;
+}
+__device__ __forceinline__ bool t16_plan_cell(const T16PlanArgs &a, const int cell, const double *mono) {
+    bool out;
+    {
         const int kc = cell / a.N_T, n = cell - kc * a.N_T, M = a.L + 1;
         const double *G = a.gram + (size_t)kc * (M * M + M), *kap = G + M * M;
         double e[9];
@@ -117,11 +150,20 @@
                 out = !(rs <= T16_PLAN_RS);
                 if (out) sq = 0;
             }
-            const bool cert = a.cert && t16_certified(a.cert + (size_t)kc * (a.n8 + a.n6), a.cert_exp, a.n8, a.n6, a.L, e + 1, dt, sq);
+            bool cert = false;
+            if (a.cert && mono)
+                cert = t16_certified_mono(a.cert + (size_t)kc * (a.n8 + a.n6), mono, a.n8, a.n6, dt, sq);
+            else if (a.cert)
+                cert = t16_certified(a.cert + (size_t)kc * (a.n8 + a.n6), a.cert_exp, a.n8, a.n6, a.L, e + 1, dt, sq);
             if (cert) a.verdict[cell] = 0;
             a.splan[cell] = sq | (cert ? T16_PLAN_CERT : 0);
         }
     }
+    return out;
+}
+__global__ void __launch_bounds__(256) t16_plan_kernel(T16PlanArgs a) {
+    const int cell = blockIdx.x * 256 + threadIdx.x;
+    const bool out = cell < a.KC * a.N_T && t16_plan_cell(a, cell, nullptr);
     const unsigned long long m = __ballot(out);
     if ((threadIdx.x & 63) == 0 && m) atomicAdd(&a.flags[6], (int)__popcll(m));
 }
@@ -134,14 +176,14 @@
     int per_traj;
     const int *rep;
 };
-__device__ __forceinline__ void ctrl_sum_body(CtrlSumArgs a) {
-    const int blk = blockIdx.x, kc = a.per_traj ? blk / a.N_T : 0, n = blk - kc * a.N_T;
+__device__ __forceinline__ void ctrl_sum_part(CtrlSumArgs a, const int blk, const int part, const int nparts) {
+    const int kc = a.per_traj ? blk / a.N_T : 0, n = blk - kc * a.N_T;
     if (a.per_traj) a.Hcf += (size_t)(a.rep ? a.rep[kc] : kc) * a.L * a.pp2;
     double e[8];
     for (int l = 0; l < a.L; ++l) e[l] = a.eps[(size_t)l * a.N_T + n] * (a.shape ? a.shape[(size_t)l * a.N_T + n] : 1.0);
     double2 *dst = (double2 *)(a.Sf + (size_t)blk * a.pp2);
 #pragma unroll 4
-    for (int i = blockIdx.y * blockDim.x + threadIdx.x; i < a.pp2 / 2; i += gridDim.y * blockDim.x) {
+    for (int i = part * blockDim.x + threadIdx.x; i < a.pp2 / 2; i += nparts * blockDim.x) {
         double2 acc = make_double2(0., 0.);
         for (int l = 0; l < a.L; ++l) {
             const double2 h = ((const double2 *)(a.Hcf + (size_t)l * a.pp2))[i];
@@ -150,6 +192,7 @@
         dst[i] = acc;
     }
 }
+__device__ __forceinline__ void ctrl_sum_body(CtrlSumArgs a) { ctrl_sum_part(a, blockIdx.x, blockIdx.y, gridDim.y); }
 __global__ void __launch_bounds__(256) ctrl_sum_kernel(CtrlSumArgs a) { ctrl_sum_body(a); }
 
 __global__ void __launch_bounds__(256) dte_kernel(const double *eps, const double *shape, const double *dts, int L, int N_T, int slots, double *out) {
@@ -1908,17 +1951,21 @@
     double *rho;
     double2 *z;
 };
+__device__ __forceinline__ double2 chi_coeff_z(const ChiCoeffArgs &a, const SweepArgs &s, const int k, double &rho) {
+    double cr, ci;
+    chi_coefficient(s, k, cr, ci);
+    const double tn = 1.0 / a.s.inv_tnorm[k];
+    rho = sqrt(cr * cr + ci * ci) * tn;
+    return make_double2(cr * tn, -ci * tn);
+}
 __device__ __forceinline__ void chi_coeff_body(const ChiCoeffArgs &a) {
     const int k = blockIdx.x * blockDim.x + threadIdx.x;
     if (k >= a.s.K) return;
     SweepArgs s = a.s;
     s.unit_chi = 0;
-    double cr, ci;
-    chi_coefficient(s, k, cr, ci);
-    const double tn = 1.0 / a.s.inv_tnorm[k];
-    const double rho = sqrt(cr * cr + ci * ci) * tn;
+    double rho;
+    a.z[k] = chi_coeff_z(a, s, k, rho);
     a.rho[k] = rho;
-    a.z[k] = make_double2(cr * tn, -ci * tn);
     if (rho < a.s.chi_min_norm) atomicOr(&a.s.flags[0], 2);
 }
 __global__ void chi_coeff_kernel(ChiCoeffArgs a) { chi_coeff_body(a); }
@@ -2975,15 +3022,18 @@
     double sub_theta;
     int *batch_flag, *flags;
 };
-__global__ void deriv_flag_kernel(DerivFlagArgs a) {
-    const int batch = blockIdx.x * blockDim.x + threadIdx.x;
-    if (batch >= a.nbatch_total) return;
+__device__ __forceinline__ bool deriv_flag_batch(const DerivFlagArgs &a, const int batch) {
     const int k = batch / a.batches_per_k, n0 = (batch - k * a.batches_per_k) * 16;
     int ns = 1;
     for (int n = n0; n < min(n0 + 16, a.N_T); ++n)
         ns = max(ns, deriv_substeps(a.rb, a.rb_k, a.sub_theta, k, a.hc_per_traj, a.L, a.eps, a.shape, a.N_T, n, a.dts[n]));
     a.batch_flag[batch] = ns > 1;
-    if (ns > 1) atomicAdd(&a.flags[3], 1);
+    return ns > 1;
+}
+__global__ void deriv_flag_kernel(DerivFlagArgs a) {
+    const int batch = blockIdx.x * blockDim.x + threadIdx.x;
+    if (batch >= a.nbatch_total) return;
+    if (deriv_flag_batch(a, batch)) atomicAdd(&a.flags[3], 1);
 }
 
 struct DerivEconArgs {
@@ -2993,9 +3043,7 @@
     int deg0, deg1;
     int *batch_econ;
 };
-__global__ void deriv_econ_kernel(DerivEconArgs a) {
-    const int batch = blockIdx.x * blockDim.x + threadIdx.x;
-    if (batch >= a.nbatch_total) return;
+__device__ __forceinline__ void deriv_econ_batch(const DerivEconArgs &a, const int batch) {
     const int k = batch / a.batches_per_k, n0 = (batch - k * a.batches_per_k) * 16;
     const int kc = a.cls ? a.cls[k] : k;
     bool ok = a.cell_deg || !t16_skipped(a.flags, a.KC * a.N_T);
@@ -3012,6 +3060,51 @@
         deg = max(deg, d);
     }
     a.batch_econ[batch] = ok ? deg : 0;
+}
+__global__ void deriv_econ_kernel(DerivEconArgs a) {
+    const int batch = blockIdx.x * blockDim.x + threadIdx.x;
+    if (batch >= a.nbatch_total) return;
+    deriv_econ_batch(a, batch);
+}
+
+struct EvalPrologueArgs {
+    CtrlSumArgs cs;
+    T16PlanArgs pl;
+    DerivFlagArgs fl;
+    int *prog;
+    int nprog;
+    int sum_x, sum_parts;
+    int plan_blocks, flag_blocks;
+};
+__global__ void __launch_bounds__(256) eval_prologue_kernel(EvalPrologueArgs a) {
+    __shared__ double plan_lds[9 * T16_PLAN_PW_LMAX + T16_PLAN_MONO_MAX];
+    int b = blockIdx.x;
+    if (b < a.plan_blocks) {
+        const bool tabled = a.pl.cert && a.pl.splan && a.pl.L <= T16_PLAN_PW_LMAX && a.pl.n8 + a.pl.n6 <= T16_PLAN_MONO_MAX;
+        if (tabled) t16_plan_monomials(a.pl, b, plan_lds);
+        for (int kc0 = 0; kc0 < a.pl.KC; kc0 += 256) {
+            const int kc = kc0 + threadIdx.x;
+            const bool out = kc < a.pl.KC && t16_plan_cell(a.pl, kc * a.pl.N_T + b, tabled ? plan_lds + 9 * T16_PLAN_PW_LMAX : nullptr);
+            const unsigned long long m = __ballot(out);
+            if ((threadIdx.x & 63) == 0 && m) atomicAdd(&a.pl.flags[6], (int)__popcll(m));
+        }
+        return;
+    }
+    b -= a.plan_blocks;
+    if (b < a.flag_blocks) {
+        const int batch = b * 256 + threadIdx.x;
+        const bool f = batch < a.fl.nbatch_total && deriv_flag_batch(a.fl, batch);
+        const unsigned long long m = __ballot(f);
+        if ((threadIdx.x & 63) == 0 && m) atomicAdd(&a.fl.flags[3], (int)__popcll(m));
+        return;
+    }
+    b -= a.flag_blocks;
+    if (b == 0) {
+        for (int i = threadIdx.x; i < a.nprog; i += 256) a.prog[i] = 0;
+        return;
+    }
+    b -= 1;
+    ctrl_sum_part(a.cs, b % a.sum_x, b / a.sum_x, a.sum_parts);
 }
 
 struct DerivSubArgs {
@@ -3682,3 +3775,42 @@
     }
 }
 __global__ void __launch_bounds__(256) grad_reduce_kernel(double2 *tg, int K, int LN, double *G, const double2 *z) { grad_reduce_body(tg, K, LN, G, z); }
+__global__ void __launch_bounds__(256) grad_reduce_chi_kernel(double2 *tg, int K, int LN, double *G, ChiCoeffArgs ca) {
+    __shared__ double part[16][17];
+    __shared__ double2 zs[1024];
+    const int j = threadIdx.x & 15, kg = threadIdx.x >> 4;
+    const int idx = blockIdx.x * 16 + j;
+    SweepArgs sc = ca.s;
+    sc.unit_chi = 0;
+    double s = 0.;
+    for (int k0 = 0; k0 < K; k0 += 1024) {
+        if (k0) __syncthreads();
+        for (int k = k0 + threadIdx.x; k < min(k0 + 1024, K); k += 256) {
+            double rho;
+            const double2 zk = chi_coeff_z(ca, sc, k, rho);
+            zs[k - k0] = zk;
+            if (blockIdx.x == 0) {
+                ca.rho[k] = rho;
+                ca.z[k] = zk;
+                if (rho < ca.s.chi_min_norm) atomicOr(&ca.s.flags[0], 2);
+            }
+        }
+        __syncthreads();
+        if (idx < LN) {
+            for (int k = k0 + kg; k < min(k0 + 1024, K); k += 16) {
+                const double2 t = tg[(size_t)k * LN + idx], zk = zs[k - k0];
+                const double2 v = make_double2(zk.x * t.x - zk.y * t.y, zk.x * t.y + zk.y * t.x);
+                tg[(size_t)k * LN + idx] = v;
+                s += v.x;
+            }
+        }
+    }
+    part[kg][j] = s;
+    __syncthreads();
+    if (kg == 0 && idx < LN) {
+        double t = 0.;
+#pragma unroll
+        for (int q = 0; q < 16; ++q) t += part[q][j];
+        G[idx] = -2.0 * t;
+    }
+}
diff --git a/grape.jl_amd/csrc/grape_t18.hip b/grape.jl_amd/csrc/grape_t18.hip
--- a/grape.jl_amd/csrc/grape_t18.hip
+++ b/grape.jl_amd/csrc/grape_t18.hip
@@ -158,6 +158,47 @@
             stat_add(a.stats, 15, (unsigned long long)__popcll(m_ok));
         }
         atomicAdd(&a.flags[5], (int)__popcll(m_valid));
+    }
+}
+
+__global__ void __launch_bounds__(256) t16_post_econ_kernel(ExpmArgs a, const int *verdict, const int *prog, int nprog, const int *splan,
+                                                             int post_blocks, DerivEconArgs ec) {
+    __shared__ unsigned long long red[4][4];
+    const int tid = threadIdx.x, lane = tid & 63, wave = tid >> 6, ncell = a.K * a.N_T;
+    if ((int)blockIdx.x >= post_blocks) {
+        const int batch = ((int)blockIdx.x - post_blocks) * 256 + tid;
+        if (batch < ec.nbatch_total) deriv_econ_batch(ec, batch);
+        return;
+    }
+    if (t16_skipped(a.flags, ncell)) return;
+    unsigned long long mi = 0, n_valid = 0, n_ok = 0, sq_ok = 0;
+    if (prog && blockIdx.x == 0)
+        for (int i = tid; i < nprog; i += 256) mi += (unsigned long long)prog[i] * 4ull * 2ull;
+#pragma unroll
+    for (int j = 0; j < 4; ++j) {
+        const int cell = blockIdx.x * 1024 + j * 256 + tid;
+        if (cell < ncell) {
+            const bool ok = verdict[cell] == 0;
+            const unsigned long long sq = (unsigned long long)(splan[cell] & T16_PLAN_SQ_MASK);
+            if (!ok) a.cell_list[atomicAdd(&a.flags[4], 1)] = cell;
+            mi += 4ull * (unsigned long long)(T16Count<4>::CELL + 1) + sq * 4ull * 192ull;
+            n_valid += 1ull;
+            if (ok) { n_ok += 1ull; sq_ok += sq; }
+        }
+    }
+    for (int off = 32; off >= 1; off >>= 1) {
+        mi += __shfl_xor(mi, off, 64); n_valid += __shfl_xor(n_valid, off, 64);
+        n_ok += __shfl_xor(n_ok, off, 64); sq_ok += __shfl_xor(sq_ok, off, 64);
+    }
+    if (lane == 0) { red[wave][0] = mi; red[wave][1] = n_valid; red[wave][2] = n_ok; red[wave][3] = sq_ok; }
+    __syncthreads();
+    if (tid == 0) {
+        unsigned long long t[4];
+        for (int q = 0; q < 4; ++q) t[q] = red[0][q] + red[1][q] + red[2][q] + red[3][q];
+        if (t[0]) stat_add(a.stats, 12, t[0]);
+        if (t[3]) stat_add(a.stats, 13, t[3]);
+        if (t[2]) { stat_add(a.stats, 14, t[2]); stat_add(a.stats, 15, t[2]); }
+        if (t[1]) atomicAdd(&a.flags[5], (int)t[1]);
     }
 }
 
@@ -426,8 +467,8 @@
 }
 
 extern "C" int grape_t16_asm_launch(const void *args, size_t args_size, int *verdict, void *stream, int blocks,
-                                    const void *const *walk, int fuse, int K) {
-    if (args_size != sizeof(ExpmArgs)) return (int)hipErrorInvalidValue;
+                                    const void *const *walk, int fuse, int K, int chain, const void *econ, size_t econ_size) {
+    if (args_size != sizeof(ExpmArgs) || (econ && econ_size != sizeof(DerivEconArgs))) return (int)hipErrorInvalidValue;
     ExpmArgs a;
     memcpy(&a, args, sizeof(a));
     if (!a.Sf || !verdict || blocks < 1 || !walk || !walk[0] || !walk[5]) return (int)hipErrorInvalidValue;
@@ -451,6 +492,14 @@
     hipStream_t s = (hipStream_t)stream;
     e = hipModuleLaunchKernel(fn, (unsigned)blocks, 1, 1, 256, 1, 1, 0, s, nullptr, cfg);
     if (e != hipSuccess) return (int)e;
+    if (chain) {
+        DerivEconArgs ec{};
+        if (econ) memcpy(&ec, econ, sizeof(ec));
+        const int post_blocks = (int)((ncell + 1023) / 1024), econ_blocks = econ ? (ec.nbatch_total + 255) / 256 : 0;
+        hipLaunchKernelGGL(t16_post_econ_kernel, dim3((unsigned)(post_blocks + econ_blocks)), dim3(256), 0, s, a, (const int *)verdict,
+                           fuse ? (const int *)walk[4] : (const int *)nullptr, 2 * K, (const int *)walk[5], post_blocks, ec);
+        return (int)hipGetLastError();
+    }
     hipLaunchKernelGGL(t16_post_kernel, dim3((unsigned)((ncell + 255) / 256)), dim3(256), 0, s, a, (const int *)verdict,
                        fuse ? (const int *)walk[4] : (const int *)nullptr, 2 * K, (const int *)walk[5]);
     return (int)hipGetLastError();
```

Measured after the change: 54.99 (median of 6 runs). No clear change (+0.3%).
